# OpenGene/repaq

Hardware: AMD Instinct MI355X
Metric: raw FASTQ MB/s encode+decode (higher is better)
Workload: dtype u8; 1 GPU; configs[2]: synthetic NovaSeq PE150 two files (-i/-I), 2 x 4.01 GB FASTQ (fqgen profile 1, 11200000 pairs, seed 3, N 20 ppm), -k 1000, encode + decode; chunks_per_gpu=3360, parity=unchecked (checked with --full)

## Files before the change

include/rfq_hip.h:

```cpp
#ifndef RFQ_HIP_H
#define RFQ_HIP_H
#include <stddef.h>
#include <stdint.h>
#ifdef __cplusplus
extern "C" {
#endif

#define RFQ_OK              0
#define RFQ_E_NO_DEVICE    -1
#define RFQ_E_HIP          -2
#define RFQ_E_ARG          -3
#define RFQ_E_TEXT         -4
#define RFQ_E_DATA         -5
#define RFQ_E_FORMAT       -6
#define RFQ_E_UNPINNED     -7
#define RFQ_E_NOSPACE      -8
#define RFQ_E_STATE        -9

#define RFQ_SE             0
#define RFQ_PE_TWO_FILES   1
#define RFQ_PE_INTERLEAVED 2

#define RFQ_HEADER_MAX     (17 + 255)

typedef struct rfq_ctx rfq_ctx;

#define RFQ_API __attribute__((visibility("default")))

RFQ_API int         rfq_create(rfq_ctx** out, int device_id);
RFQ_API void        rfq_destroy(rfq_ctx* ctx);
RFQ_API const char* rfq_last_error(const rfq_ctx* ctx);
RFQ_API int         rfq_set_stream(rfq_ctx* ctx, void* hip_stream);

RFQ_API int rfq_set_header(rfq_ctx* ctx, const uint8_t* h_header, size_t header_len);
RFQ_API int rfq_get_header(rfq_ctx* ctx, uint8_t* h_out , size_t* header_len);
RFQ_API void rfq_clear_header(rfq_ctx* ctx);

typedef struct {
    const uint8_t* d_fq1; size_t n1;
    const uint8_t* d_fq2; size_t n2;
    int32_t  paired;
    uint32_t chunk_bases;
    int32_t  final;
    int32_t  emit_header;
    uint64_t file_off1, file_off2;
    uint64_t nolb_from1, nolb_from2;
    uint8_t* d_out; size_t out_cap;
    int32_t  flush_all;
    uint32_t carry_bases;
} rfq_encode_args;

typedef struct {
    const uint8_t* d_rfq;
    size_t   rfq_len;
    uint32_t n_chunks;
    uint64_t n_reads;
    uint64_t n_bases;
    size_t   consumed1, consumed2;
    const uint64_t* h_chunk_off;
    int32_t  input_ended;
    int32_t  reserved;
} rfq_encode_result;

RFQ_API int rfq_encode_batch(rfq_ctx* ctx, const rfq_encode_args* args, rfq_encode_result* res);

typedef struct {
    uint32_t n_chunks;
    uint64_t n_reads;
    size_t   consumed1, consumed2;
    const uint64_t* h_end1;
    const uint64_t* h_end2;
    int32_t  input_ended;
    uint32_t unit_bases;
} rfq_scan_result;
RFQ_API int rfq_scan_batch(rfq_ctx* ctx, const rfq_encode_args* args, rfq_scan_result* res);

typedef struct {
    const uint8_t* d_rfq; size_t n;
    int32_t  has_header;
    int32_t  split_pe;
    int32_t  final;
    int32_t  bug_compat;
    uint8_t* d_out1; size_t cap1;
    uint8_t* d_out2; size_t cap2;
    const uint64_t* h_chunk_off; uint32_t n_chunk_off; uint32_t reserved3;
} rfq_decode_args;

typedef struct {
    const uint8_t* d_fq1; size_t n1;
    const uint8_t* d_fq2; size_t n2;
    uint32_t n_chunks;
    uint64_t n_reads, n_bases;
    size_t   consumed;
} rfq_decode_result;

RFQ_API int rfq_decode_batch(rfq_ctx* ctx, const rfq_decode_args* args, rfq_decode_result* res);

#define RFQ_ROWS_ASCII 0
#define RFQ_ROWS_CODE  1
typedef struct {
    const uint8_t* d_rfq; size_t n;
    int32_t  has_header, final;
    const uint64_t* h_chunk_off; uint32_t n_chunk_off;
    uint32_t row_len;
    int32_t  base_mode;
    uint8_t  qual_offset;
    uint8_t  pad_base, pad_qual;
    uint8_t  reserved;
    uint8_t* d_bases; size_t bases_cap;
    uint8_t* d_quals; size_t quals_cap;
    int32_t* d_lens;  size_t lens_cap;
} rfq_decode_rows_args;
typedef struct {
    uint64_t n_rows, n_bases;
    uint32_t n_chunks, max_len;
    size_t   consumed;
} rfq_decode_rows_result;
RFQ_API int rfq_decode_rows(rfq_ctx* ctx, const rfq_decode_rows_args* args, rfq_decode_rows_result* res);

typedef struct {
    uint64_t n_rows;
    uint32_t row_len;
    int32_t  base_mode;
    uint8_t  qual_offset;
    uint8_t  reserved[3];
    const uint8_t* d_bases;
    const uint8_t* d_quals;
    const int32_t* d_lens;
    const uint8_t* d_names; size_t names_len;
    const uint64_t* d_name_off;
} rfq_rows_in;
typedef struct {
    const uint8_t* d_fq1; size_t n1;
    const uint8_t* d_fq2; size_t n2;
    uint64_t n_reads, n_bases;
} rfq_rows_text_result;
RFQ_API int rfq_rows_to_text(rfq_ctx* ctx, const rfq_rows_in* rows, int32_t paired, uint8_t* d_out1, size_t cap1, uint8_t* d_out2, size_t cap2,
                             int32_t size_only, rfq_rows_text_result* res);
RFQ_API int rfq_encode_rows(rfq_ctx* ctx, const rfq_rows_in* rows, const rfq_encode_args* enc, rfq_encode_result* res);

RFQ_API int rfq_last_timings(const rfq_ctx* ctx, const char** names, float* ms, int cap);

RFQ_API int rfq_dev_malloc(rfq_ctx* ctx, void** d_ptr, size_t n);
RFQ_API int rfq_dev_free(rfq_ctx* ctx, void* d_ptr);
RFQ_API int rfq_copy_h2d(rfq_ctx* ctx, void* d_dst, const void* h_src, size_t n);
RFQ_API int rfq_copy_h2d_async(rfq_ctx* ctx, void* d_dst, const void* h_src, size_t n, uint64_t* ticket);
RFQ_API int rfq_copy_done(rfq_ctx* ctx, uint64_t ticket);
RFQ_API int rfq_copy_sync(rfq_ctx* ctx);
RFQ_API int rfq_copy_d2h(rfq_ctx* ctx, void* h_dst, const void* d_src, size_t n);
RFQ_API int rfq_copy_d2d(rfq_ctx* ctx, void* d_dst, const void* d_src, size_t n);
RFQ_API int rfq_copy_peer(rfq_ctx* ctx, void* d_dst, const rfq_ctx* src_ctx, const void* d_src, size_t n);
RFQ_API int rfq_host_alloc(rfq_ctx* ctx, void** h_ptr, size_t n);
RFQ_API int rfq_host_free(rfq_ctx* ctx, void* h_ptr);
RFQ_API int rfq_host_register(rfq_ctx* ctx, void* h_ptr, size_t n);
RFQ_API int rfq_host_unregister(rfq_ctx* ctx, void* h_ptr);

RFQ_API int rfq_compare_bytes(rfq_ctx* ctx, const void* d_a, const void* d_b, size_t n, uint64_t* first_diff);

RFQ_API int rfq_set_option(rfq_ctx* ctx, const char* name, const char* value);
RFQ_API int rfq_get_option(const rfq_ctx* ctx, const char* name, char* out, size_t cap);
RFQ_API const char* rfq_option_name(int i);

RFQ_API int rfq_selftest_wave(rfq_ctx* ctx, const uint64_t* h_in, uint32_t n_waves, uint64_t* h_out);

RFQ_API const char* rfq_version(void);

#ifdef __cplusplus
}
#endif
#endif
```

repaq_amd/_capi.py:

```python
import ctypes as C
import os

_HERE = os.path.dirname(os.path.abspath(__file__))
DEFAULT_LIB = os.path.join(_HERE, "lib", "librfq_hip.so")

RFQ_OK = 0
SE, PE_TWO_FILES, PE_INTERLEAVED = 0, 1, 2
HEADER_MAX = 17 + 255
U64_MAX = (1 << 64) - 1
ERRORS = {-1: "RFQ_E_NO_DEVICE", -2: "RFQ_E_HIP", -3: "RFQ_E_ARG", -4: "RFQ_E_TEXT", -5: "RFQ_E_DATA", -6: "RFQ_E_FORMAT",
          -7: "RFQ_E_UNPINNED", -8: "RFQ_E_NOSPACE", -9: "RFQ_E_STATE"}


class RfqError(RuntimeError):
    def __init__(self, code, msg):
        super().__init__("%s: %s" % (ERRORS.get(code, code), msg))
        self.code = code
        self.message = msg


class EncodeArgs(C.Structure):
    _fields_ = [("d_fq1", C.c_void_p), ("n1", C.c_size_t), ("d_fq2", C.c_void_p), ("n2", C.c_size_t), ("paired", C.c_int32),
                ("chunk_bases", C.c_uint32), ("final", C.c_int32), ("emit_header", C.c_int32), ("file_off1", C.c_uint64),
                ("file_off2", C.c_uint64), ("nolb_from1", C.c_uint64), ("nolb_from2", C.c_uint64), ("d_out", C.c_void_p), ("out_cap", C.c_size_t),
                ("flush_all", C.c_int32), ("carry_bases", C.c_uint32)]


class EncodeResult(C.Structure):
    _fields_ = [("d_rfq", C.c_void_p), ("rfq_len", C.c_size_t), ("n_chunks", C.c_uint32), ("n_reads", C.c_uint64), ("n_bases", C.c_uint64),
                ("consumed1", C.c_size_t), ("consumed2", C.c_size_t), ("h_chunk_off", C.POINTER(C.c_uint64)),
                ("input_ended", C.c_int32), ("reserved", C.c_int32)]


class ScanResult(C.Structure):
    _fields_ = [("n_chunks", C.c_uint32), ("n_reads", C.c_uint64), ("consumed1", C.c_size_t), ("consumed2", C.c_size_t),
                ("h_end1", C.POINTER(C.c_uint64)), ("h_end2", C.POINTER(C.c_uint64)), ("input_ended", C.c_int32), ("unit_bases", C.c_uint32)]


class DecodeArgs(C.Structure):
    _fields_ = [("d_rfq", C.c_void_p), ("n", C.c_size_t), ("has_header", C.c_int32), ("split_pe", C.c_int32), ("final", C.c_int32), ("bug_compat", C.c_int32),
                ("d_out1", C.c_void_p), ("cap1", C.c_size_t), ("d_out2", C.c_void_p), ("cap2", C.c_size_t),
                ("h_chunk_off", C.POINTER(C.c_uint64)), ("n_chunk_off", C.c_uint32), ("reserved3", C.c_uint32)]


class DecodeResult(C.Structure):
    _fields_ = [("d_fq1", C.c_void_p), ("n1", C.c_size_t), ("d_fq2", C.c_void_p), ("n2", C.c_size_t), ("n_chunks", C.c_uint32),
                ("n_reads", C.c_uint64), ("n_bases", C.c_uint64), ("consumed", C.c_size_t)]


ROWS_ASCII, ROWS_CODE = 0, 1


class DecodeRowsArgs(C.Structure):
    _fields_ = [("d_rfq", C.c_void_p), ("n", C.c_size_t), ("has_header", C.c_int32), ("final", C.c_int32),
                ("h_chunk_off", C.POINTER(C.c_uint64)), ("n_chunk_off", C.c_uint32), ("row_len", C.c_uint32), ("base_mode", C.c_int32),
                ("qual_offset", C.c_uint8), ("pad_base", C.c_uint8), ("pad_qual", C.c_uint8), ("reserved", C.c_uint8),
                ("d_bases", C.c_void_p), ("bases_cap", C.c_size_t), ("d_quals", C.c_void_p), ("quals_cap", C.c_size_t),
                ("d_lens", C.c_void_p), ("lens_cap", C.c_size_t)]


class DecodeRowsResult(C.Structure):
    _fields_ = [("n_rows", C.c_uint64), ("n_bases", C.c_uint64), ("n_chunks", C.c_uint32), ("max_len", C.c_uint32), ("consumed", C.c_size_t)]


class RowsIn(C.Structure):
    _fields_ = [("n_rows", C.c_uint64), ("row_len", C.c_uint32), ("base_mode", C.c_int32), ("qual_offset", C.c_uint8), ("reserved", C.c_uint8 * 3),
                ("d_bases", C.c_void_p), ("d_quals", C.c_void_p), ("d_lens", C.c_void_p), ("d_names", C.c_void_p), ("names_len", C.c_size_t),
                ("d_name_off", C.c_void_p)]


class RowsTextResult(C.Structure):
    _fields_ = [("d_fq1", C.c_void_p), ("n1", C.c_size_t), ("d_fq2", C.c_void_p), ("n2", C.c_size_t), ("n_reads", C.c_uint64), ("n_bases", C.c_uint64)]


_libs = {}


def load(path=None):
    path = path or os.environ.get("RFQ_HIP_LIBRARY") or DEFAULT_LIB
    if path in _libs:
        return _libs[path]
    try:
        import torch
    except Exception:
        pass
    if not os.path.exists(path):
        raise ImportError("librfq_hip.so not found at %s — build it with `python -c 'import __graft_entry__ as g; g.build()'` "
                          "(hipcc --offload-arch=gfx950); repaq_amd has no CPU fallback" % path)
    L = C.CDLL(path)
    L.rfq_version.restype = C.c_char_p
    L.rfq_create.argtypes = [C.POINTER(C.c_void_p), C.c_int]
    L.rfq_destroy.argtypes = [C.c_void_p]
    L.rfq_last_error.argtypes = [C.c_void_p]; L.rfq_last_error.restype = C.c_char_p
    L.rfq_set_stream.argtypes = [C.c_void_p, C.c_void_p]
    L.rfq_set_header.argtypes = [C.c_void_p, C.c_char_p, C.c_size_t]
    L.rfq_get_header.argtypes = [C.c_void_p, C.c_char_p, C.POINTER(C.c_size_t)]
    L.rfq_clear_header.argtypes = [C.c_void_p]; L.rfq_clear_header.restype = None
    L.rfq_encode_batch.argtypes = [C.c_void_p, C.POINTER(EncodeArgs), C.POINTER(EncodeResult)]
    L.rfq_decode_batch.argtypes = [C.c_void_p, C.POINTER(DecodeArgs), C.POINTER(DecodeResult)]
    L.rfq_decode_rows.argtypes = [C.c_void_p, C.POINTER(DecodeRowsArgs), C.POINTER(DecodeRowsResult)]
    L.rfq_rows_to_text.argtypes = [C.c_void_p, C.POINTER(RowsIn), C.c_int32, C.c_void_p, C.c_size_t, C.c_void_p, C.c_size_t, C.c_int32, C.POINTER(RowsTextResult)]
    L.rfq_encode_rows.argtypes = [C.c_void_p, C.POINTER(RowsIn), C.POINTER(EncodeArgs), C.POINTER(EncodeResult)]
    L.rfq_scan_batch.argtypes = [C.c_void_p, C.POINTER(EncodeArgs), C.POINTER(ScanResult)]
    L.rfq_last_timings.argtypes = [C.c_void_p, C.POINTER(C.c_char_p), C.POINTER(C.c_float), C.c_int]
    L.rfq_dev_malloc.argtypes = [C.c_void_p, C.POINTER(C.c_void_p), C.c_size_t]
    L.rfq_dev_free.argtypes = [C.c_void_p, C.c_void_p]
    L.rfq_copy_h2d.argtypes = [C.c_void_p, C.c_void_p, C.c_char_p, C.c_size_t]
    L.rfq_copy_h2d_async.argtypes = [C.c_void_p, C.c_void_p, C.c_void_p, C.c_size_t, C.POINTER(C.c_uint64)]
    L.rfq_copy_done.argtypes = [C.c_void_p, C.c_uint64]
    L.rfq_copy_sync.argtypes = [C.c_void_p]
    L.rfq_copy_d2h.argtypes = [C.c_void_p, C.c_void_p, C.c_void_p, C.c_size_t]
    L.rfq_copy_d2d.argtypes = [C.c_void_p, C.c_void_p, C.c_void_p, C.c_size_t]
    L.rfq_copy_peer.argtypes = [C.c_void_p, C.c_void_p, C.c_void_p, C.c_void_p, C.c_size_t]
    L.rfq_host_alloc.argtypes = [C.c_void_p, C.POINTER(C.c_void_p), C.c_size_t]
    L.rfq_host_free.argtypes = [C.c_void_p, C.c_void_p]
    L.rfq_compare_bytes.argtypes = [C.c_void_p, C.c_void_p, C.c_void_p, C.c_size_t, C.POINTER(C.c_uint64)]
    L.rfq_set_option.argtypes = [C.c_void_p, C.c_char_p, C.c_char_p]
    L.rfq_get_option.argtypes = [C.c_void_p, C.c_char_p, C.c_char_p, C.c_size_t]
    L.rfq_option_name.argtypes = [C.c_int]; L.rfq_option_name.restype = C.c_char_p
    L.rfq_selftest_wave.argtypes = [C.c_void_p, C.POINTER(C.c_uint64), C.c_uint32, C.POINTER(C.c_uint64)]
    _libs[path] = L
    return L


EXPORTS = ["rfq_version", "rfq_create", "rfq_destroy", "rfq_last_error", "rfq_set_stream", "rfq_set_header", "rfq_get_header", "rfq_clear_header",
           "rfq_encode_batch", "rfq_scan_batch", "rfq_decode_batch", "rfq_decode_rows", "rfq_rows_to_text", "rfq_encode_rows", "rfq_last_timings", "rfq_dev_malloc", "rfq_dev_free", "rfq_copy_h2d", "rfq_copy_d2h",
           "rfq_copy_h2d_async", "rfq_copy_done", "rfq_copy_sync",
           "rfq_copy_d2d", "rfq_copy_peer", "rfq_host_alloc", "rfq_host_free", "rfq_compare_bytes", "rfq_selftest_wave", "rfq_set_option", "rfq_get_option", "rfq_option_name", "rfq_host_register", "rfq_host_unregister"]
```

repaq_amd/codec.py:

```python
import ctypes as C

from . import _capi as A
from ._capi import RfqError, SE, PE_TWO_FILES, PE_INTERLEAVED, U64_MAX


class RfqCodec:
    def __init__(self, device=0, library=None):
        self._L = A.load(library)
        h = C.c_void_p()
        rc = self._L.rfq_create(C.byref(h), device)
        if rc != A.RFQ_OK:
            raise RfqError(rc, "rfq_create(device=%d) failed: no usable MI355X / HIP device (there is no CPU fallback)" % device)
        self._h = h

    def close(self):
        if getattr(self, "_h", None):
            self._L.rfq_destroy(self._h)
            self._h = None

    __del__ = close

    def _check(self, rc):
        if rc != A.RFQ_OK:
            raise RfqError(rc, self._L.rfq_last_error(self._h).decode("latin-1"))

    def version(self):
        return self._L.rfq_version().decode()

    def set_stream(self, stream_ptr):
        self._check(self._L.rfq_set_stream(self._h, stream_ptr))

    def set_option(self, name, value=None):
        self._check(self._L.rfq_set_option(self._h, name.encode(), None if value is None else str(value).encode()))

    def get_option(self, name) -> str:
        buf = C.create_string_buffer(64)
        self._check(self._L.rfq_get_option(self._h, name.encode(), buf, 64))
        return buf.value.decode()

    def option_names(self):
        out, i = [], 0
        while True:
            n = self._L.rfq_option_name(i)
            if not n:
                return out
            out.append(n.decode()); i += 1

    def option(self, name, value):
        import contextlib

        @contextlib.contextmanager
        def scope():
            before = self.get_option(name)
            self.set_option(name, value)
            try:
                yield self
            finally:
                self.set_option(name, before or None)
        return scope()

    def selftest_wave(self, lanes):
        n = len(lanes); assert n and n % 64 == 0
        a = (C.c_uint64 * n)(*lanes); o = (C.c_uint64 * (12 * n))()
        self._check(self._L.rfq_selftest_wave(self._h, a, n // 64, o))
        return [list(o[12 * i: 12 * i + 12]) for i in range(n)]

    def setHeader(self, header_bytes: bytes):
        self._check(self._L.rfq_set_header(self._h, header_bytes, len(header_bytes)))

    def clearHeader(self):
        self._L.rfq_clear_header(self._h)

    def header(self) -> bytes:
        buf = C.create_string_buffer(A.HEADER_MAX); n = C.c_size_t()
        self._check(self._L.rfq_get_header(self._h, buf, C.byref(n)))
        return buf.raw[: n.value]

    def encode(self, d_fq1, n1, d_fq2=None, n2=0, paired=SE, chunk_bases=1_000_000, final=True, emit_header=True,
               file_off1=0, file_off2=0, nolb_from1=U64_MAX, nolb_from2=U64_MAX, d_out=None, out_cap=0, flush_all=False):
        a = A.EncodeArgs(d_fq1, n1, d_fq2, n2, paired, chunk_bases, 1 if final else 0, 1 if emit_header else 0,
                         file_off1, file_off2, nolb_from1, nolb_from2, d_out, out_cap, 1 if flush_all else 0, 0)
        r = A.EncodeResult()
        self._check(self._L.rfq_encode_batch(self._h, C.byref(a), C.byref(r)))
        return r

    def scan(self, d_fq1, n1, d_fq2=None, n2=0, paired=SE, chunk_bases=1_000_000, final=True, file_off1=0, file_off2=0, carry_bases=0):
        a = A.EncodeArgs(d_fq1, n1, d_fq2, n2, paired, chunk_bases, 1 if final else 0, 0, file_off1, file_off2, U64_MAX, U64_MAX, None, 0, 0, carry_bases)
        r = A.ScanResult()
        self._check(self._L.rfq_scan_batch(self._h, C.byref(a), C.byref(r)))
        ends1 = [r.h_end1[i] for i in range(r.n_chunks)]
        ends2 = [r.h_end2[i] for i in range(r.n_chunks)] if (paired == PE_TWO_FILES and r.n_chunks) else []
        return r, ends1, ends2

    def decode(self, d_rfq, n, has_header=True, split_pe=False, final=True, d_out1=None, cap1=0, d_out2=None, cap2=0, chunk_off=None, n_chunks=0, bug_compat=False):
        if chunk_off is not None and not isinstance(chunk_off, C.POINTER(C.c_uint64)):
            n_chunks = len(chunk_off) - 1
            chunk_off = C.cast((C.c_uint64 * len(chunk_off))(*chunk_off), C.POINTER(C.c_uint64))
        a = A.DecodeArgs(d_rfq, n, 1 if has_header else 0, 1 if split_pe else 0, 1 if final else 0, 1 if bug_compat else 0, d_out1, cap1, d_out2, cap2,
                         chunk_off if (chunk_off is not None and n_chunks) else None, n_chunks if chunk_off is not None else 0, 0)
        r = A.DecodeResult()
        self._check(self._L.rfq_decode_batch(self._h, C.byref(a), C.byref(r)))
        return r

    def decode_rows(self, d_rfq, n, row_len=0, codes=False, qual_offset=33, pad_base=255, pad_qual=255, d_bases=None, bases_cap=0, d_quals=None, quals_cap=0,
                    d_lens=None, lens_cap=0, has_header=True, final=True, chunk_off=None, n_chunks=0):
        if chunk_off is not None and not isinstance(chunk_off, C.POINTER(C.c_uint64)):
            n_chunks = len(chunk_off) - 1
            chunk_off = C.cast((C.c_uint64 * len(chunk_off))(*chunk_off), C.POINTER(C.c_uint64))
        a = A.DecodeRowsArgs(d_rfq, n, 1 if has_header else 0, 1 if final else 0, chunk_off if (chunk_off is not None and n_chunks) else None,
                             n_chunks if chunk_off is not None else 0, row_len, A.ROWS_CODE if codes else A.ROWS_ASCII, qual_offset, pad_base, pad_qual, 0,
                             d_bases, bases_cap, d_quals, quals_cap, d_lens, lens_cap)
        r = A.DecodeRowsResult()
        self._check(self._L.rfq_decode_rows(self._h, C.byref(a), C.byref(r)))
        return r

    def decode_rows_bytes(self, rfq: bytes, row_len=None, codes=False, qual_offset=33, pad_base=255, pad_qual=255, bases=True, quals=True, lens=True, **kw):
        import numpy as np
        d = self.dev_put(rfq); bufs = []
        try:
            q = self.decode_rows(d, len(rfq), **kw)
            L = max(q.max_len, 1) if row_len is None else int(row_len)
            n = q.n_rows; nb = max(n * L, 1)
            ob = self.dev_put(b"\0" * nb) if bases else None
            oq = self.dev_put(b"\0" * nb) if quals else None
            ol = self.dev_put(b"\0" * max(4 * n, 4)) if lens else None
            bufs = [x for x in (ob, oq, ol) if x is not None]
            r = self.decode_rows(d, len(rfq), row_len=L, codes=codes, qual_offset=qual_offset, pad_base=pad_base, pad_qual=pad_qual,
                                 d_bases=ob, bases_cap=n * L, d_quals=oq, quals_cap=n * L, d_lens=ol, lens_cap=n, **kw)
            n = r.n_rows

            def rows(p):
                return np.frombuffer(self.dev_get(p, n * L), dtype=np.uint8).reshape(n, L) if p is not None else None
            lv = np.frombuffer(self.dev_get(ol, 4 * n), dtype=np.int32) if ol is not None else None
            return n, r.max_len, rows(ob), rows(oq), lv
        finally:
            self.dev_free(d)
            for p in bufs:
                self.dev_free(p)

    @staticmethod
    def _rows_in(n_rows, row_len, d_bases, d_quals, d_lens, d_names, names_len, d_name_off, codes, qual_offset):
        return A.RowsIn(n_rows, row_len, A.ROWS_CODE if codes else A.ROWS_ASCII, qual_offset, (C.c_uint8 * 3)(), d_bases, d_quals, d_lens, d_names, names_len, d_name_off)

    def rows_to_text(self, n_rows, row_len, d_bases, d_quals, d_lens, d_names, names_len, d_name_off, paired=SE, codes=False, qual_offset=33,
                     d_out1=None, cap1=0, d_out2=None, cap2=0, size_only=False):
        a = self._rows_in(n_rows, row_len, d_bases, d_quals, d_lens, d_names, names_len, d_name_off, codes, qual_offset)
        r = A.RowsTextResult()
        self._check(self._L.rfq_rows_to_text(self._h, C.byref(a), paired, d_out1, cap1, d_out2, cap2, 1 if size_only else 0, C.byref(r)))
        return r

    def encode_rows(self, n_rows, row_len, d_bases, d_quals, d_lens, d_names, names_len, d_name_off, paired=SE, codes=False, qual_offset=33,
                    chunk_bases=1_000_000, final=True, emit_header=True, file_off1=0, file_off2=0, nolb_from1=U64_MAX, nolb_from2=U64_MAX,
                    d_out=None, out_cap=0, flush_all=False, d_fq1=None):
        a = self._rows_in(n_rows, row_len, d_bases, d_quals, d_lens, d_names, names_len, d_name_off, codes, qual_offset)
        e = A.EncodeArgs(d_fq1, 0, None, 0, paired, chunk_bases, 1 if final else 0, 1 if emit_header else 0,
                         file_off1, file_off2, nolb_from1, nolb_from2, d_out, out_cap, 1 if flush_all else 0, 0)
        r = A.EncodeResult()
        self._check(self._L.rfq_encode_rows(self._h, C.byref(a), C.byref(e), C.byref(r)))
        return r

    def _put_rows(self, bases, quals, lens, names):
        import numpy as np
        bases = np.ascontiguousarray(bases, dtype=np.uint8); quals = np.ascontiguousarray(quals, dtype=np.uint8)
        lens = np.ascontiguousarray(lens, dtype=np.int32)
        n = int(lens.shape[0]); L = int(bases.shape[1]) if bases.ndim == 2 else 0
        assert bases.shape == quals.shape == (n, L) and len(names) == n and L >= 1, "bases / quals [n, L], lens [n], n names"
        off = np.zeros(n + 1, dtype=np.uint64)
        if n:
            off[1:] = np.cumsum(np.fromiter((len(x) for x in names), dtype=np.uint64, count=n))
        blob = b"".join(names)
        ptrs = [self.dev_put(x) for x in (bases.tobytes(), quals.tobytes(), lens.tobytes(), blob, off.tobytes())]
        return ptrs, (n, L, ptrs[0], ptrs[1], ptrs[2], ptrs[3], len(blob), ptrs[4])

    def rows_to_text_bytes(self, bases, quals, lens, names, paired=SE, codes=False, qual_offset=33):
        ptrs, rows = self._put_rows(bases, quals, lens, names)
        try:
            r = self.rows_to_text(*rows, paired=paired, codes=codes, qual_offset=qual_offset)
            a = self.dev_get(r.d_fq1, r.n1) if r.n1 else b""
            b = self.dev_get(r.d_fq2, r.n2) if (paired == PE_TWO_FILES and r.n2) else b""
            return (a, b) if paired == PE_TWO_FILES else a
        finally:
            for p in ptrs:
                self.dev_free(p)

    def encode_rows_bytes(self, bases, quals, lens, names, paired=SE, chunk_bases=1_000_000, codes=False, qual_offset=33, **kw) -> bytes:
        ptrs, rows = self._put_rows(bases, quals, lens, names)
        try:
            r = self.encode_rows(*rows, paired=paired, codes=codes, qual_offset=qual_offset, chunk_bases=chunk_bases, **kw)
            return self.dev_get(r.d_rfq, r.rfq_len) if r.rfq_len else b""
        finally:
            for p in ptrs:
                self.dev_free(p)

    def first_diff(self, d_a, d_b, n) -> int:
        out = C.c_uint64(0)
        self._check(self._L.rfq_compare_bytes(self._h, d_a, d_b, n, C.byref(out)))
        return out.value

    def timings(self):
        names = (C.c_char_p * 32)(); ms = (C.c_float * 32)()
        n = self._L.rfq_last_timings(self._h, names, ms, 32)
        return [(names[i].decode(), ms[i]) for i in range(n)]

    def dev_put(self, data: bytes):
        p = C.c_void_p()
        self._check(self._L.rfq_dev_malloc(self._h, C.byref(p), max(len(data), 1) + 64))
        self._check(self._L.rfq_copy_h2d(self._h, p, data, len(data)))
        return p

    def dev_get(self, d_ptr, n) -> bytes:
        buf = C.create_string_buffer(max(n, 1))
        self._check(self._L.rfq_copy_d2h(self._h, buf, d_ptr, n))
        return buf.raw[:n]

    def dev_free(self, p):
        self._L.rfq_dev_free(self._h, p)

    def encode_bytes(self, fq1: bytes, fq2: bytes = b"", paired=SE, chunk_bases=1_000_000, **kw) -> bytes:
        d1 = self.dev_put(fq1); d2 = self.dev_put(fq2) if paired == PE_TWO_FILES else None
        try:
            r = self.encode(d1, len(fq1), d2, len(fq2) if d2 else 0, paired, chunk_bases, **kw)
            return self.dev_get(r.d_rfq, r.rfq_len) if r.rfq_len else b""
        finally:
            self.dev_free(d1)
            if d2:
                self.dev_free(d2)

    def decode_bytes(self, rfq: bytes, split_pe=False, out_caps=None, **kw):
        d = self.dev_put(rfq); o1 = o2 = None
        try:
            if out_caps is not None:
                o1 = self.dev_put(b"\0" * max(int(out_caps[0]), 1)); o2 = self.dev_put(b"\0" * max(int(out_caps[1]), 1)) if split_pe else None
                kw = dict(kw, d_out1=o1, cap1=int(out_caps[0]), d_out2=o2, cap2=int(out_caps[1]) if split_pe else 0)
            r = self.decode(d, len(rfq), split_pe=split_pe, **kw)
            a = self.dev_get(r.d_fq1, r.n1) if r.n1 else b""
            b = self.dev_get(r.d_fq2, r.n2) if (split_pe and r.n2) else b""
            return (a, b) if split_pe else a
        finally:
            self.dev_free(d)
            if o1 is not None: self.dev_free(o1)
            if o2 is not None: self.dev_free(o2)


def nolb_threshold(file_size: int, ends_with_newline: bool) -> int:
    if file_size == 0:
        return U64_MAX
    if file_size % (1 << 20) == 0:
        return file_size
    if ends_with_newline:
        return U64_MAX
    return ((file_size - 1) >> 20) << 20
```

repaq_amd/csrc/dec/emit_tiles.h:

```cpp
#pragma once
#define E3_QCAP 10240u
#define E3_SHARED_OK 1
#define E3_ALIGNED 1
#define E3_PROBE_WRAP 0
#define E3_PREFETCH 0
#define E3_L2PF 1
#define E3_N1BIG 13312u
struct __attribute__((packed, aligned(1))) GU16d { uint32_t a, b, c, d; };
struct __attribute__((packed, aligned(1))) GU8d { uint32_t a, b; };
struct __attribute__((packed, aligned(1))) GU4d { uint32_t a; };
struct __attribute__((packed, aligned(1))) GU2d { uint16_t a; };
__device__ __forceinline__ void e3_copy(uint8_t* __restrict__ dst, const uint8_t* src, uint32_t n, uint32_t g0, uint32_t gs, int pat, uint32_t dch) {
    if (n >= 16u) {
        const uint32_t ng = (n + 15u) >> 4;
        for (uint32_t g = g0; g < ng; g += gs) {
            uint32_t p0 = 16u * g; if (p0 + 16u > n) p0 = n - 16u;
            uint32_t w[4]; lds_get16(src, p0, w);
            if (pat >= (int)p0 && pat < (int)p0 + 16) { const int b = pat - (int)p0; const uint32_t sh = 8u * (uint32_t)(b & 3); uint32_t& x = w[b >> 2];
                    x = (x & ~(0xFFu << sh)) | ((dch & 0xFFu) << sh); }
            GU16d v; v.a = w[0]; v.b = w[1]; v.c = w[2]; v.d = w[3]; *(GU16d*)(dst + p0) = v;
        }
    } else if (g0 == 0 && n) {
        uint32_t w[4]; lds_get16(src, 0, w);
        if (pat >= 0 && pat < 16) { const uint32_t sh = 8u * (uint32_t)(pat & 3); uint32_t& x = w[pat >> 2]; x = (x & ~(0xFFu << sh)) | ((dch & 0xFFu) << sh); }
        uint8_t* q = dst;
        if (n & 8u) { GU8d v; v.a = w[0]; v.b = w[1]; *(GU8d*)q = v; q += 8; w[0] = w[2]; w[1] = w[3]; }
        if (n & 4u) { GU4d v; v.a = w[0]; *(GU4d*)q = v; q += 4; w[0] = w[1]; }
        if (n & 2u) { GU2d v; v.a = (uint16_t)w[0]; *(GU2d*)q = v; q += 2; w[0] >>= 16; }
        if (n & 1u) *q = (uint8_t)w[0];
    }
}
__device__ __forceinline__ uint32_t e3_rev2x16(uint32_t v) { v = bswap32(v); v = ((v >> 4) & 0x0F0F0F0Fu) | ((v & 0x0F0F0F0Fu) << 4);
        return ((v >> 2) & 0x33333333u) | ((v & 0x33333333u) << 2); }
__device__ __forceinline__ uint32_t e3_rev1x16(uint32_t v) {
    v = ((v >> 8) & 0xFFu) | ((v & 0xFFu) << 8); v = ((v >> 4) & 0x0F0Fu) | ((v & 0x0F0Fu) << 4);
    v = ((v >> 2) & 0x3333u) | ((v & 0x3333u) << 2); return ((v >> 1) & 0x5555u) | ((v & 0x5555u) << 1);
}
__device__ __forceinline__ uint32_t e3_from(int t, int i) { const int k = t - 4 * i; return k <= 0 ? 0xFFFFFFFFu : (k >= 4 ? 0u : 0xFFFFFFFFu << (8 * k)); }
__device__ __forceinline__ uint32_t e3_align(uint32_t hi, uint32_t lo, int bytes) { return (uint32_t)((((unsigned long long)hi << 32) | lo) >> (8 * bytes)); }
template <bool IMPL, uint32_t N1CAP = ET_N1CAP, bool SHARED = false> __global__ void __launch_bounds__(256, (N1CAP == ET_N1CAP && !(SHARED && E3_PREFETCH)) ? 5 : 4) k_dec_emit3(const uint8_t* __restrict__ img,
        const DChunk* __restrict__ CH, const DevHeader* __restrict__ D, DFused F,
                           uint64_t img_bytes, int split, uint8_t* __restrict__ out1, uint64_t cap1, uint8_t* __restrict__ out2, uint64_t cap2, DecStatus* st,
                           const plist_t* __restrict__ plist, const unsigned long long* __restrict__ loff, const uint32_t* __restrict__ nent, const uint32_t* __restrict__ cellidx,
                           uint32_t ncell, uint32_t nstr, uint32_t kshift, unsigned long long list_cap) {
    __shared__ uint4 t_q4[E3_QCAP / 16 + 6];
    constexpr uint32_t NB = (SHARED && E3_PREFETCH) ? 2u : 1u;
    __shared__ uint4 t_pk4[NB][E3_QCAP / 64 + 6];
    __shared__ uint32_t t_nb[E3_QCAP / 32 + 8];
    __shared__ uint4 t_mid4_[NB][64 * E3_MIDROW / 16 + 5], t_n14_[(SHARED ? 256u : N1CAP) / 16 + 5], t_n24_[(SHARED ? 256u : ET_N2CAP) / 16 + 5], t_st4[(SHARED ? 256u : ET_STCAP) / 16 + 4];
    uint4* const t_n14 = t_n14_ + 1; uint4* const t_n24 = t_n24_ + 1;
    __shared__ unsigned long long s_loff[NPOS_SLOT + 2]; __shared__ uint32_t s_nent[NPOS_SLOT + 2], s_val[NPOS_SLOT + 2];
    __shared__ uint32_t s_g[2][NPOS_SLOT + 2], s_kb[2][NPOS_SLOT + 2];
    const uint32_t c = blockIdx.y; const DChunk d = CH[c]; const uint8_t* cp = img + d.off;
    const uint32_t fl = d.flags, hf = D->flags, f = d.rbase; const bool il = (fl & C_PE_INTERLEAVED) != 0;
    constexpr bool implied_n = IMPL;
    const uint32_t nq4 = (D->n_base_qual & 0xFFu) * 0x01010101u, dpos = D->name2_diff_pos, dch = D->name2_diff_char;
    const int l = lane_id(), w = (int)uni32((uint32_t)wave_id()); const uint32_t tid = threadIdx.x;
    const size_t fp = (size_t)f + c;
    const U4 tb = F.tbase[c];
    const uint32_t K = 1u << kshift, pshift = 8u - kshift, P = 1u << pshift;
    uint32_t per = (d.reads + gridDim.x - 1) / gridDim.x; per = (per + K - 1u) & ~(K - 1u);
    const uint32_t rs = blockIdx.x * per; const uint32_t re = rs + per < d.reads ? rs + per : d.reads;
    if (rs >= re) return;
    if (list_cap && ((st->err & (uint32_t)(DE_CORRUPT | DE_CORRUPT_OV | DE_LIST_ALIAS | DE_E3_RETRY)) || st->list_need > list_cap)) return;
    const bool raw = !SHARED && (hf & H_DONT_QUAL) != 0, bycol = SHARED || (!raw && (hf & H_QUAL_BY_COL));
    const uint32_t nn = bycol ? (D->n_normal < NPOS_SLOT ? D->n_normal : NPOS_SLOT) : 0u; const bool hasn = (hf & H_N_POS) != 0;
    const uint32_t T = nn + (hasn ? 1u : 0u);
    const uint32_t major4 = (D->major & 0xFFu) * 0x01010101u;
    const uint32_t qlen_c = F.pql[fp + d.reads], slen_c = F.sdl[fp + d.reads];
    const bool same1 = SHARED || (fl & C_NAME1_SAME) != 0, same2 = SHARED || (fl & C_NAME2_SAME) != 0, same3 = SHARED || (fl & C_STRAND_SAME) != 0;
    if (tid < T) { const uint32_t jj = tid < nn ? tid : D->n_normal; const size_t t_ = (size_t)c * nstr + jj; s_loff[tid] = loff[t_]; s_nent[tid] = nent[t_];
            s_val[tid] = tid < nn ? (uint32_t)D->normal[tid] : (uint32_t)'N'; }
    uint32_t nrec = 0; const uint8_t* xrec = nullptr;
    if (bycol && 4ull * D->n_normal <= d.qual_size) {
        const uint8_t* qp = cp + d.o_qual; uint64_t off = 4ull * D->n_normal;
        for (uint32_t i = 0; i < D->n_normal; i++) off += ld_u32(qp + 4 * i);
        off = uni64(off);
        if (off <= d.qual_size) { nrec = (uint32_t)((d.qual_size - off) / 5); xrec = qp + off; }
    }
    auto cell_lookup = [&](uint32_t t, uint32_t qpos, uint32_t spos, bool bound) -> uint32_t {
        const uint32_t jj = t < nn ? t : D->n_normal; uint32_t cell = ((t < nn ? qpos : spos) + (bound ? E3_QCAP : 0u)) / POS2_CELL + (bound ? 1u : 0u);
        if (cell >= ncell) return bound ? 0xFFFFFFFFu : cellidx[((size_t)c * nstr + jj) * ncell + ncell - 1u];
        return cellidx[((size_t)c * nstr + jj) * ncell + cell];
    };
    struct TileP { uint32_t q0, q1, s0, s1, a7, a8, a9, e7, e8, e9; };
    auto tile_params = [&](uint32_t r0, uint32_t r1) -> TileP {
        TileP t; t.q0 = uni32(F.pql[fp + r0]); t.q1 = uni32(F.pql[fp + r1]);
        t.s0 = uni32(F.sdl[fp + r0]); t.s1 = uni32(F.sdl[fp + r1]);
        if constexpr (SHARED) { t.a7 = t.a8 = t.a9 = t.e7 = t.e8 = t.e9 = 0u; }
        else { const U4 a = F.pvl[fp + r0], b = F.pvl[fp + r1];
               t.a7 = uni32(a.a); t.a8 = uni32(a.b); t.a9 = uni32(a.c); t.e7 = uni32(b.a); t.e8 = uni32(b.b); t.e9 = uni32(b.c); }
        return t;
    };
    constexpr bool PF = SHARED && E3_PREFETCH;
    uint32_t cur = rs, pb = 0; uint32_t l2pf = 0; (void)l2pf;
    TileP tp_cur = tile_params(cur, cur + K < re ? cur + K : re);
    if (tid < T) { s_g[0][tid] = cell_lookup(tid, tp_cur.q0, tp_cur.s0, false); s_kb[0][tid] = cell_lookup(tid, tp_cur.q0, tp_cur.s0, true); }
    {
        const uint64_t ib = d.off;
        if (same1) span_dma<1>(make_span(t_n14, img, ib + d.o_n1, ib + d.o_n1 + d.n1_size, img_bytes, true));
        if (same2) span_dma<1>(make_span(t_n24, img, ib + d.o_n2, ib + d.o_n2 + d.n2_size, img_bytes, true));
        if (same3) span_dma<1>(make_span(t_st4, img, ib + d.o_st, ib + d.o_st + d.st_size, img_bytes, true));
    }
    const uint32_t jj = tid >> pshift, j = ((jj << 1) & (K - 1u)) | (jj >> (kshift - 1u)), part = tid & (P - 1u);
    struct TileD { uint64_t n1a, n1e, n2a, n2e, sta, ste, pka, pke, rqa, rqe; };
    auto tile_spans = [&](const TileP& tp) -> TileD {
        TileD t; const uint64_t ib = d.off;
        t.n1a = ib + d.o_n1 + (same1 ? 0u : tp.a7); t.n1e = same1 ? t.n1a + d.n1_size : ib + d.o_n1 + tp.e7;
        t.n2a = ib + d.o_n2 + (same2 ? 0u : tp.a8); t.n2e = same2 ? t.n2a + d.n2_size : ib + d.o_n2 + tp.e8;
        t.sta = ib + d.o_st + (same3 ? 0u : tp.a9); t.ste = same3 ? t.sta + d.st_size : ib + d.o_st + tp.e9;
        t.pka = ib + d.o_seq + (tp.s0 >> 2); t.pke = ib + d.o_seq + ((tp.s1 + 3u) >> 2); { const uint64_t pend = ib + d.o_seq + d.seq_size; if (t.pke > pend) t.pke = pend;
                if (t.pka > t.pke) t.pka = t.pke; }
        t.rqa = ib + d.o_qual + tp.q0; t.rqe = ib + d.o_qual + tp.q1; { const uint64_t qend = ib + d.o_qual + d.qual_size; if (t.rqe > qend) t.rqe = qend;
                if (t.rqa > t.rqe) t.rqa = t.rqe; }
        return t;
    };
    auto tile_fits = [&](const TileP& tp) -> bool {
        return tp.q1 - tp.q0 <= E3_QCAP && (same1 || tp.e7 - tp.a7 + 32u <= N1CAP) && (same2 || tp.e8 - tp.a8 + 32u <= ET_N2CAP) && (same3 || tp.e9 - tp.a9 + 32u <= ET_STCAP);
    };
    auto stage = [&](const TileD& t, uint32_t g0_, uint32_t g1_, uint32_t bsel) {
        if (raw) span_dma<(int)((E3_QCAP / 16 + 4 + 255) / 256)>(make_span(t_q4 + 1, img, t.rqa, t.rqe, img_bytes, true));
        if (w == 0) span_dma_wave<(int)((E3_QCAP / 64 + 4 + 63) / 64), PF>(make_span(t_pk4[bsel], img, t.pka, t.pke, img_bytes, true), l);
        else if (w == 1) span_dma_wave<(int)((64 * E3_MIDROW / 16 + 4 + 63) / 64), PF>(make_span(t_mid4_[bsel] + 1, F.mid, (uint64_t)g0_ * E3_MIDROW, (uint64_t)g1_ * E3_MIDROW, ~0ull >> 1, true), l);
        else if (w == 2) { if (!same1) span_dma_wave<(int)((N1CAP / 16 + 4 + 63) / 64)>(make_span(t_n14, img, t.n1a, t.n1e, img_bytes, true), l); }
        else { if (!same2) span_dma_wave<(int)((ET_N2CAP / 16 + 4 + 63) / 64)>(make_span(t_n24, img, t.n2a, t.n2e, img_bytes, true), l);
               if (!same3) span_dma_wave<(int)((ET_STCAP / 16 + 4 + 63) / 64)>(make_span(t_st4, img, t.sta, t.ste, img_bytes, true), l); }
    };
    struct ReadM { uint32_t len, md, prevlen, sdl, pql, tx; int ov; U4 p4; uint8_t n1, n2, sl; };
    auto load_read = [&](uint32_t cur_, uint32_t cnt_) -> ReadM {
        ReadM m; m.len = m.n1 = m.n2 = m.sl = m.md = m.prevlen = m.sdl = m.pql = m.tx = 0; m.ov = 0; m.p4.a = m.p4.b = m.p4.c = m.p4.d = 0;
        const uint32_t r = cur_ + j;
        if (j < cnt_) {
            const uint32_t g_ = f + r; const uint2 t2 = F.tpl[g_];
            m.sdl = F.sdl[fp + r];
            if constexpr (!SHARED) m.p4 = F.pvl[fp + r];
            m.tx = t2.x; m.pql = F.pql[fp + r];
            m.len = F.len[g_]; m.ov = F.ov[g_]; m.prevlen = (r & 1u) ? F.len[g_ - 1] : 0u;
            m.n1 = cp[d.o_n1lens + ((fl & C_NAME1_LEN_SAME) ? 0u : r)]; m.n2 = (hf & H_NAME2) ? cp[d.o_n2lens + ((fl & C_NAME2_LEN_SAME) ? 0u : r)] : 0u;
            m.sl = cp[d.o_stlens + ((fl & C_STRAND_LEN_SAME) ? 0u : r)]; m.md = t2.y;
        }
        return m;
    };
    struct ListS { uint32_t fe[8], fv[8], pn[2], nk0, nke, t, base, k0, ke, val; const plist_t* p; };
    auto ls_open = [&](ListS& L, uint32_t pb_, uint32_t t_) {
        const uint32_t g_ = uni32(s_g[pb_][t_]), b_ = uni32(s_kb[pb_][t_]), n_ = uni32(s_nent[t_]);
        L.k0 = g_ == 0xFFFFFFFFu ? 0u : g_; L.ke = g_ == 0xFFFFFFFFu ? 0u : (b_ < n_ ? b_ : n_); L.base = 0;
        L.val = uni32(s_val[t_]); L.p = plist + uni64(s_loff[t_]);
    };
    auto ls_round = [&](ListS& L, uint32_t pb_, uint32_t& e_, uint32_t& v_) {
        while (L.t < nn && L.k0 + L.base >= L.ke) { L.t += 4u; if (L.t < nn) ls_open(L, pb_, L.t); }
        if (L.t < nn) { const uint32_t kk = L.k0 + L.base + (uint32_t)l; if (kk < L.ke) e_ = L.p[kk]; v_ = L.val; L.base += 64u; }
    };
    auto load_lists = [&](uint32_t pb_) -> ListS {
        ListS L; L.t = (uint32_t)w; L.base = L.k0 = L.ke = L.val = 0; L.p = plist;
        if (L.t < nn) ls_open(L, pb_, L.t); else L.t = nn;
#pragma unroll
        for (int i = 0; i < 8; i++) { L.fe[i] = 0xFFFFFFFFu; L.fv[i] = 0; ls_round(L, pb_, L.fe[i], L.fv[i]); }
        L.pn[0] = L.pn[1] = 0xFFFFFFFFu; L.nk0 = 0xFFFFFFFFu; L.nke = 0;
        if (hasn) {
            L.nk0 = s_g[pb_][nn]; L.nke = s_kb[pb_][nn]; if (L.nke > s_nent[nn]) L.nke = s_nent[nn];
            const plist_t* lp = plist + s_loff[nn];
#pragma unroll
            for (int i = 0; i < 2; i++) { const uint32_t kk = L.nk0 + tid + 256u * (uint32_t)i; if (L.nk0 != 0xFFFFFFFFu && kk < L.nke) L.pn[i] = lp[kk]; }
        }
        return L;
    };
    __syncthreads();
    ReadM mN; ListS lN;
    if constexpr (PF) {
        if (tile_fits(tp_cur)) { const uint32_t cnt0 = re - cur < K ? re - cur : K; stage(tile_spans(tp_cur), f + cur, f + cur + cnt0, 0u); mN = load_read(cur, cnt0); lN = load_lists(0u); }
        else { mN = load_read(cur, 0u); lN = load_lists(0u); }
    }
    while (cur < re) {
        const uint32_t cnt = re - cur < K ? re - cur : K, g0 = f + cur, g1 = g0 + cnt;
        const TileP tp = tp_cur; const uint32_t q0 = tp.q0, q1 = tp.q1, s0 = tp.s0, s1 = tp.s1;
        if (!tile_fits(tp)) { if (tid == 0) atomicOr(&st->err, (uint32_t)DE_E3_RETRY); break; }
        const TileD td = tile_spans(tp); const uint32_t bs = PF ? pb : 0u;
        const uint64_t n1a = td.n1a, n2a = td.n2a, sta = td.sta, pka = td.pka, pke = td.pke, rqa = td.rqa;
        if constexpr (!PF) { stage(td, g0, g1, 0u); mN = load_read(cur, cnt); lN = load_lists(pb); }
        const ReadM m = mN; ListS ls = lN;
        if (bycol) { uint4* qt = t_q4 + 1; const uint32_t ng = (q1 - q0 + 15u) >> 4;
                for (uint32_t i = tid; i < ng; i += blockDim.x) qt[i] = make_uint4(major4, major4, major4, major4); }
        for (uint32_t i = tid; i < ((s1 - s0 + 31u) >> 5) + 1u; i += blockDim.x) t_nb[i] = 0;
        const uint32_t r = cur + j; const bool on = j < cnt; const bool odd = (r & 1u) != 0, rc = il && odd, to2 = split && odd;
        const uint32_t len = m.len, n1 = m.n1, n2 = m.n2, sl = m.sl, md = m.md, prevlen = m.prevlen; const int ov = m.ov;
        uint32_t sp = 0, qp_ = 0, o7 = 0, o8 = 0, o9 = 0, toff = 0;
        if (on) { sp = m.sdl - s0; qp_ = m.pql - q0; toff = (to2 ? tb.b : tb.a) + m.tx; if constexpr (!SHARED) { o7 = m.p4.a - tp.a7; o8 = m.p4.b - tp.a8; o9 = m.p4.c - tp.a9; } }
        const uint32_t nxt = cur + cnt; TileP tp_n = tp;
        if (nxt < re) tp_n = tile_params(nxt, nxt + K < re ? nxt + K : re);
#ifndef RFQ_SIMT_EMULATION
        if constexpr (PF) __builtin_amdgcn_s_waitcnt(0x0F70);
#endif
        __syncthreads();
#if E3_L2PF && !defined(RFQ_SIMT_EMULATION)
        if (SHARED) asm volatile("" :: "v"(l2pf));
#endif
        uint8_t* const q_t = (uint8_t*)(t_q4 + 1) + (raw ? (uint32_t)(rqa & 15ull) : 0u);
        const uint8_t* const pk = (const uint8_t*)t_pk4[bs] + (uint32_t)(pka & 15ull);
        const uint4* const t_mid4 = t_mid4_[bs] + 1;
        const uint32_t have = (uint32_t)(pke - pka), sbit0 = 2u * (s0 & 3u);
        {
#pragma unroll
            for (int i = 0; i < 8; i++) { const uint32_t p = plist_pos(ls.fe[i], q0); if (p < q1) q_t[p - q0] = (uint8_t)ls.fv[i]; }
            while (ls.t < nn) {
                uint32_t e_[4], v_[4];
#pragma unroll
                for (int i = 0; i < 4; i++) { e_[i] = 0xFFFFFFFFu; v_[i] = 0; ls_round(ls, pb, e_[i], v_[i]); }
#pragma unroll
                for (int i = 0; i < 4; i++) { const uint32_t p = plist_pos(e_[i], q0); if (p < q1) q_t[p - q0] = (uint8_t)v_[i]; }
            }
            if (nrec) for (uint32_t i = tid; i < nrec; i += blockDim.x) { const uint8_t* rr = xrec + 5ull * i; const uint32_t pos = ld_u32(rr + 1);
                    if (pos >= q0 && pos < q1 && pos < qlen_c) q_t[pos - q0] = rr[0]; }
            if (hasn) {
                const uint32_t send = s1 < slen_c ? s1 : slen_c;
#pragma unroll
                for (int i = 0; i < 2; i++) { const uint32_t p = plist_pos(ls.pn[i], s0); if (p < send) atomicOr(&t_nb[(p - s0) >> 5], 1u << ((p - s0) & 31u)); }
                if (ls.nk0 != 0xFFFFFFFFu && ls.nk0 + 512u < ls.nke) { const plist_t* lp = plist + s_loff[nn];
                        for (uint32_t kk = ls.nk0 + 512u + tid; kk < ls.nke; kk += 256u) { const uint32_t p = plist_pos((uint32_t)lp[kk], s0);
                        if (p < send) atomicOr(&t_nb[(p - s0) >> 5], 1u << ((p - s0) & 31u)); } }
            }
        }
        if (nxt < re && tid < T) { s_g[pb ^ 1u][tid] = cell_lookup(tid, tp_n.q0, tp_n.s0, false); s_kb[pb ^ 1u][tid] = cell_lookup(tid, tp_n.q0, tp_n.s0, true); }
        __syncthreads();
        if constexpr (PF) {
            if (nxt < re) {
                const uint32_t cntn = re - nxt < K ? re - nxt : K;
                if (tile_fits(tp_n)) { stage(tile_spans(tp_n), f + nxt, f + nxt + cntn, pb ^ 1u); mN = load_read(nxt, cntn); lN = load_lists(pb ^ 1u); }
            }
        }
#if E3_L2PF && !defined(RFQ_SIMT_EMULATION)
        if (SHARED && nxt < re) {
            const uint32_t cntn = re - nxt < K ? re - nxt : K; const TileD tn = tile_spans(tp_n);
            const uint8_t* pb_ = nullptr; uint32_t nbytes = 0;
            const uint32_t grp = tid >> 5, li = tid & 31u; uint32_t line = li;
            if (grp == 0) { pb_ = img + tn.pka; nbytes = (uint32_t)(tn.pke - tn.pka); }
            else if (grp == 1) { pb_ = F.mid + (size_t)(f + nxt) * E3_MIDROW; nbytes = cntn * E3_MIDROW; }
            else if (grp == 2) {
                const uint32_t a = li >> 2; line = li & 3u;
                if (a == 0) { pb_ = (const uint8_t*)(F.tpl + f + nxt); nbytes = cntn * 8u; }
                else if (a == 1) { pb_ = (const uint8_t*)(F.sdl + fp + nxt); nbytes = cntn * 4u; }
                else if (a == 2) { pb_ = (const uint8_t*)(F.pql + fp + nxt); nbytes = cntn * 4u; }
                else if (a == 3) { pb_ = (const uint8_t*)(F.len + f + nxt); nbytes = cntn * 4u; }
                else if (a == 4) { pb_ = (const uint8_t*)(F.ov + f + nxt); nbytes = cntn * 4u; }
            }
            else {
                const uint32_t t_ = grp - 3u, st_ = t_ < 4u ? t_ : nn;
                if ((t_ < 4u && t_ < nn) || (t_ == 4u && hasn)) {
                    const uint32_t g_ = s_g[pb ^ 1u][st_], b_ = s_kb[pb ^ 1u][st_], n_ = s_nent[st_]; const uint32_t ke = b_ < n_ ? b_ : n_;
                    if (g_ != 0xFFFFFFFFu && g_ < ke) { pb_ = (const uint8_t*)(plist + s_loff[st_] + g_); nbytes = (ke - g_) * (uint32_t)sizeof(plist_t); }
                }
            }
            if (nbytes) {
                const uint8_t* const a0 = (const uint8_t*)((uintptr_t)pb_ & ~(uintptr_t)127); const uint32_t span = (uint32_t)(pb_ - a0) + nbytes;
                if (128u * line < span) { const uint8_t* q = a0 + 128u * line; asm volatile("global_load_dword %0, %1, off" : "=v"(l2pf) : "v"(q)); }
            }
        }
#endif
        if (on) {
            uint8_t* const rec = (to2 ? out2 : out1) + (E3_PROBE_WRAP ? (toff & (uint32_t)E3_PROBE_WRAP) : toff); const uint64_t capo = to2 ? cap2 : cap1;
            const uint32_t e0 = n1 + md + n2, oseq = e0 + 1u, ost = oseq + len + 1u, oq = ost + sl + 1u, total = oq + len + 1u;
            if ((uint64_t)toff + total > capo) { if (part == 0) atomicOr(&st->err, 1u << 31); }
            else {
                const uint32_t L = e0 + 1u; const bool nfast = L >= 16u, jfast = sl == 1u && len >= 16u;
                const uint8_t* const src1 = (const uint8_t*)t_n14 + (uint32_t)(n1a & 15ull) + (same1 ? 0u : o7);
                const uint8_t* const src2 = (const uint8_t*)t_mid4 + (uint32_t)(((uint64_t)g0 * E3_MIDROW) & 15ull) + E3_MIDROW * j;
                const uint8_t* const src3 = (const uint8_t*)t_n24 + (uint32_t)(n2a & 15ull) + (same2 ? 0u : o8);
                const uint8_t* const src4 = (const uint8_t*)t_st4 + (uint32_t)(sta & 15ull) + (same3 ? 0u : o9);
                const int pat2 = (same2 && rc && dch != 0 && dpos < n2) ? (int)dpos : -1;
                if (nfast) {
                    const uint32_t ngl = (L + 15u) >> 4;
                    for (uint32_t gi = part; gi < ngl; gi += P) {
                        uint32_t p0 = 16u * gi; if (p0 + 16u > L) p0 = L - 16u;
                        const int t1 = (int)n1 - (int)p0, t2 = t1 + (int)md, t3 = t2 + (int)n2;
                        uint32_t w[4] = { 0, 0, 0, 0 }, x[4];
                        if (t1 > 0) lds_get16(src1 + p0, 0, w);
                        if (t1 < 16 && t2 > 0 && md) { lds_get16(src2 - t1, 0, x);
#pragma unroll
                            for (int i = 0; i < 4; i++) { const uint32_t m = e3_from(t1, i); w[i] = (w[i] & ~m) | (x[i] & m); } }
                        if (t2 < 16 && t3 > 0 && n2) { lds_get16(src3 - t2, 0, x);
                            if (pat2 >= 0) { const int b = t2 + pat2; if (b >= 0 && b < 16) { const uint32_t sh = 8u * (uint32_t)(b & 3); uint32_t& y = x[b >> 2];
                                    y = (y & ~(0xFFu << sh)) | ((dch & 0xFFu) << sh); } }
#pragma unroll
                            for (int i = 0; i < 4; i++) { const uint32_t m = e3_from(t2, i); w[i] = (w[i] & ~m) | (x[i] & m); } }
                        if (t3 == 15) w[3] = (w[3] & 0x00FFFFFFu) | 0x0A000000u;
                        GU16d v; v.a = w[0]; v.b = w[1]; v.c = w[2]; v.d = w[3]; *(GU16d*)(rec + p0) = v;
                    }
                } else {
                    if (part == 0) e3_copy(rec, src1, n1, 0, 1, -1, 0);
                    else if (part == 1 % P) e3_copy(rec + n1, src2, md, 0, 1, -1, 0);
                    if (part == 2 % P) e3_copy(rec + n1 + md, src3, n2, 0, 1, pat2, dch);
                    if (part == 3 % P) rec[e0] = '\n';
                }
                if (!jfast && part == 3 % P) { e3_copy(rec + ost, src4, sl, 0, 1, -1, 0); rec[ost - 1u] = '\n'; rec[oq - 1u] = '\n'; rec[total - 1u] = '\n'; }
                const uint32_t xa = ov < 0 ? len - (uint32_t)(-ov) : len; const uint32_t A = ov > 0 ? sp - (uint32_t)ov : sp, Bs = sp - prevlen;
                auto fetch = [&](uint32_t si, uint32_t& cw, uint32_t& nw) {
                    const uint32_t bit = sbit0 + 2u * si, byte = bit >> 3; const unsigned long long v = lds_get8(pk, byte);
                    cw = (uint32_t)(v >> (bit & 7u));
                    const uint32_t nb_ = lds_get4((const uint8_t*)t_nb, (si >> 3)) >> (si & 7u); nw = nb_ & 0xFFFFu;
                    if (byte + 5u > have) { uint32_t lim_ = 4u * have > sbit0 / 2u + si ? 4u * have - sbit0 / 2u - si : 0u;
                            if (lim_ < 16u) nw |= (0xFFFFu << lim_) & 0xFFFFu; }
                };
                auto group_q = [&](uint32_t k0, uint32_t (&qw)[4]) {
                    const uint32_t pa = rc ? len - k0 - 16u : k0;
                    lds_get16(q_t, qp_ + pa, qw);
                    if (rc) { const uint32_t x0 = bswap32(qw[3]), x1 = bswap32(qw[2]), x2 = bswap32(qw[1]), x3 = bswap32(qw[0]); qw[0] = x0; qw[1] = x1; qw[2] = x2; qw[3] = x3; }
                };
                auto group_s = [&](uint32_t k0, const uint32_t (&qw)[4], uint32_t (&sw)[4]) {
                    const uint32_t pa = rc ? len - k0 - 16u : k0;
                    uint32_t cw, nw;
                    if (pa + 16u <= xa) fetch(A + pa, cw, nw);
                    else if (pa >= xa) fetch(Bs + (pa - xa), cw, nw);
                    else { uint32_t c2, n2_; const uint32_t t1 = xa - pa; fetch(A + pa, cw, nw); fetch(Bs, c2, n2_);
                            cw = (cw & ((1u << (2u * t1)) - 1u)) | (c2 << (2u * t1)); nw = (nw & ((1u << t1) - 1u)) | ((n2_ << t1) & 0xFFFFu); }
                    if (rc) { cw = ~e3_rev2x16(cw); if (nw) nw = e3_rev1x16(nw); }
#pragma unroll
                    for (int i = 0; i < 4; i++) { const uint32_t b = (cw >> (8 * i)) & 0xFFu, y = (b | (b << 12)) & 0x000F000Fu, idx = (y | (y << 6)) & 0x03030303u;
                            sw[i] = __builtin_amdgcn_perm(0u, 0x43544147u, idx); }
                    if (nw) {
#pragma unroll
                        for (int i = 0; i < 4; i++) { const uint32_t mk = ((((nw >> (4 * i)) & 0xFu) * 0x00204081u) & 0x01010101u) * 0xFFu;
                                sw[i] = (sw[i] & ~mk) | (0x4E4E4E4Eu & mk); }
                    }
                    if (implied_n) {
#pragma unroll
                        for (int i = 0; i < 4; i++) { const uint32_t mk = eq_bytes_full(qw[i], nq4); sw[i] = (sw[i] & ~mk) | (0x4E4E4E4Eu & mk); }
                    }
                };
                auto group = [&](uint32_t k0, uint32_t (&qw)[4], uint32_t (&sw)[4]) { group_q(k0, qw); group_s(k0, qw, sw); };
                auto st16 = [&](uint32_t at, const uint32_t (&x)[4]) { GU16d v; v.a = x[0]; v.b = x[1]; v.c = x[2]; v.d = x[3]; *(GU16d*)(rec + at) = v; };
                auto put = [&](uint32_t at_q, uint32_t at_s, const uint32_t (&qw)[4], const uint32_t (&sw)[4], bool both) {
                    GU16d v;
                    if (both) { v.a = qw[0]; v.b = qw[1]; v.c = qw[2]; v.d = qw[3]; *(GU16d*)(rec + at_q) = v; }
                    v.a = sw[0]; v.b = sw[1]; v.c = sw[2]; v.d = sw[3]; *(GU16d*)(rec + at_s) = v;
                };
                if (len >= 16u) {
                    uint32_t qw[4], sw[4];
                    const bool al = E3_ALIGNED && len >= 32u;
                    uint32_t rs, tail_part;
                    if (al) {
                        const uint32_t hs = (16u - (uint32_t)((uintptr_t)(rec + oseq) & 15u)) & 15u, hq = (16u - (uint32_t)((uintptr_t)(rec + oq) & 15u)) & 15u;
                        const uint32_t nts = ((len - hs) >> 4) + (hs ? 1u : 0u), ntq = ((len - hq) >> 4) + (hq ? 1u : 0u);
                        for (uint32_t t = part; t < nts; t += P) { const uint32_t k0 = hs ? (t ? hs + 16u * (t - 1u) : 0u) : 16u * t;
                                if (implied_n) group_q(k0, qw);
                                group_s(k0, qw, sw); st16(oseq + k0, sw); }
                        const uint32_t p2 = (part + P - (nts & (P - 1u))) & (P - 1u);
                        for (uint32_t t = p2; t < ntq; t += P) { const uint32_t k0 = hq ? (t ? hq + 16u * (t - 1u) : 0u) : 16u * t; group_q(k0, qw); st16(oq + k0, qw); }
                        rs = (len - hs) & 15u; tail_part = (nts + ntq) & (P - 1u);
                        if (!jfast && tail_part == part) {
                            const uint32_t rq = (len - hq) & 15u;
                            if (rs || rq) { group(len - 16u, qw, sw); if (rq) st16(oq + len - 16u, qw); if (rs) st16(oseq + len - 16u, sw); }
                        }
                    } else {
                        const uint32_t nfull = len >> 4;
                        for (uint32_t gi = part; gi < nfull; gi += P) { group(16u * gi, qw, sw); put(oq + 16u * gi, oseq + 16u * gi, qw, sw, true); }
                        rs = len & 15u; tail_part = nfull & (P - 1u);
                        if (!jfast && tail_part == part && rs) { group(len - 16u, qw, sw); put(oq + len - 16u, oseq + len - 16u, qw, sw, true); }
                    }
                    if (jfast && tail_part == part) {
                        group(len - 16u, qw, sw);
                        {
                            if (rs > 13u) put(0u, oseq + len - 16u, qw, sw, false);
                            const uint32_t jd = 0x000A000Au | ((uint32_t)src4[0] << 8);
                            uint32_t qs[4], ss[4];
                            ss[0] = e3_align(sw[1], sw[0], 3); ss[1] = e3_align(sw[2], sw[1], 3); ss[2] = e3_align(sw[3], sw[2], 3); ss[3] = e3_align(jd, sw[3], 3);
                            qs[0] = e3_align(qw[1], qw[0], 1); qs[1] = e3_align(qw[2], qw[1], 1); qs[2] = e3_align(qw[3], qw[2], 1); qs[3] = e3_align(0x0Au, qw[3], 1);
                            put(oq + len - 15u, oseq + len - 13u, qs, ss, true);
                        }
                    }
                } else if (part == 0) {
                    for (uint32_t k = 0; k < len; k++) {
                        const uint32_t p = rc ? len - 1u - k : k, si = p < xa ? A + p : Bs + (p - xa);
                        const uint32_t bit = sbit0 + 2u * si, byte = bit >> 3; const uint32_t code = byte < have ? (pk[byte] >> (bit & 7u)) & 3u : 0u;
                        const bool isn = byte >= have || ((t_nb[si >> 5] >> (si & 31u)) & 1u);
                        const uint8_t q = q_t[qp_ + p]; uint8_t b = isn ? (uint8_t)'N' : (uint8_t)("GATC"[rc ? 3u - code : code]);
                        if (implied_n && q == (uint8_t)(nq4 & 0xFFu)) b = 'N';
                        rec[oseq + k] = b; rec[oq + k] = q;
                    }
                }
            }
        }
        __syncthreads();
        cur += cnt; pb ^= 1u; tp_cur = tp_n;
    }
}
```

repaq_amd/csrc/dec/read_table.h:

```cpp
#pragma once
struct DReadTab {
    uint32_t* len; uint32_t* chunk; int32_t* ov; U4* pvin; U4* pv; uint32_t* pq; U4* tin; U4* tp;
    uint8_t* mid;
};
__device__ __forceinline__ uint32_t dec_read_len(const uint8_t* cp, const DChunk& d, uint32_t rlb, uint32_t r) {
    const uint8_t* p = cp + d.o_readlens + (size_t)((d.flags & C_READ_LEN_SAME) ? 0u : r) * rlb;
    return rlb == 1 ? p[0] : (rlb == 2 ? ld_u16(p) : ld_u32(p));
}
__global__ void k_dec_readtab(const uint8_t* __restrict__ img, const DChunk* __restrict__ CH, const DevHeader* __restrict__ D, DReadTab R, DecStatus* st) {
    const DChunk d = CH[blockIdx.y]; const uint32_t r = blockIdx.x * blockDim.x + threadIdx.x;
    if (r >= d.reads) return;
    const uint8_t* cp = img + d.off; const uint32_t g = d.rbase + r, fl = d.flags, hf = D->flags;
    const uint32_t len = dec_read_len(cp, d, D->read_len_bytes, r);
    U4 v;
    v.a = (fl & C_NAME1_SAME) ? 0u : cp[d.o_n1lens + ((fl & C_NAME1_LEN_SAME) ? 0u : r)];
    v.b = ((hf & H_NAME2) && !(fl & C_NAME2_SAME)) ? cp[d.o_n2lens + ((fl & C_NAME2_LEN_SAME) ? 0u : r)] : 0u;
    v.c = (fl & C_STRAND_SAME) ? 0u : cp[d.o_stlens + ((fl & C_STRAND_LEN_SAME) ? 0u : r)];
    int ov = 0; uint32_t stored = len;
    if ((fl & C_PE_INTERLEAVED) && (hf & H_PE_OVERLAP) && (r & 1u)) {
        ov = (int)(int8_t)cp[d.o_ov + r / 2] - D->overlap_shift;
        const uint32_t a = (uint32_t)(ov < 0 ? -ov : ov);
        const uint32_t prevlen = dec_read_len(cp, d, D->read_len_bytes, r - 1);
        if (a > len || a > prevlen) { atomicOr(&st->err, (uint32_t)DE_CORRUPT); ov = 0; } else stored = len - a;
    }
    v.d = stored;
    R.len[g] = len; R.chunk[g] = blockIdx.y; R.ov[g] = ov; R.pvin[g] = v;
}
#define E3_MIDROW 32u
struct DFused {
    const uint32_t* len; const int32_t* ov;
    const uint32_t* pql;
    const U4* pvl;
    const uint32_t* sdl;
    const uint2* tpl;
    const U4* tbase;
    const uint8_t* mid;
};
__global__ void __launch_bounds__(256) k_dec_readtab2(const uint8_t* __restrict__ img, const DChunk* __restrict__ CH, const DevHeader* __restrict__ D,
                                                      uint32_t* __restrict__ len_o, int32_t* __restrict__ ov_o, uint32_t* __restrict__ pql, U4* __restrict__ pvl, uint32_t* __restrict__ sdl, DecStatus* st) {
    const uint32_t c = blockIdx.x; const DChunk d = CH[c];
    const uint8_t* cp = img + d.off; const uint32_t fl = d.flags, hf = D->flags, rlb = D->read_len_bytes, shift = (uint32_t)D->overlap_shift;
    const bool ovl = (fl & C_PE_INTERLEAVED) && (hf & H_PE_OVERLAP);
    const size_t fp = (size_t)d.rbase + c;
    U4 carry; carry.a = carry.b = carry.c = carry.d = 0; uint32_t qcarry = 0, bad = 0;
    for (uint32_t r0 = 0; r0 < d.reads; r0 += 4u * blockDim.x) {
        const uint32_t rb = r0 + 4u * threadIdx.x;
        U4 v[4]; uint32_t ln[4]; U4 sum; sum.a = sum.b = sum.c = sum.d = 0; uint32_t qsum = 0;
#pragma unroll
        for (int i = 0; i < 4; i++) {
            const uint32_t r = rb + (uint32_t)i; v[i].a = v[i].b = v[i].c = v[i].d = 0; ln[i] = 0;
            if (r < d.reads) {
                const uint32_t len = dec_read_len(cp, d, rlb, r);
                v[i].a = (fl & C_NAME1_SAME) ? 0u : cp[d.o_n1lens + ((fl & C_NAME1_LEN_SAME) ? 0u : r)];
                v[i].b = ((hf & H_NAME2) && !(fl & C_NAME2_SAME)) ? cp[d.o_n2lens + ((fl & C_NAME2_LEN_SAME) ? 0u : r)] : 0u;
                v[i].c = (fl & C_STRAND_SAME) ? 0u : cp[d.o_stlens + ((fl & C_STRAND_LEN_SAME) ? 0u : r)];
                int ov = 0; uint32_t stored = len;
                if (ovl && (r & 1u)) {
                    ov = (int)(int8_t)cp[d.o_ov + r / 2] - (int)shift;
                    const uint32_t a = (uint32_t)(ov < 0 ? -ov : ov);
                    const uint32_t prevlen = dec_read_len(cp, d, rlb, r - 1);
                    if (a > len || a > prevlen) { bad = 1; ov = 0; } else stored = len - a;
                }
                v[i].d = stored; ln[i] = len;
                len_o[(size_t)d.rbase + r] = len; ov_o[(size_t)d.rbase + r] = ov;
            }
            sum = sum + v[i]; qsum += ln[i];
        }
        U4 tot; uint32_t qtot;
        U4 run = carry + block_excl_sum<U4>(sum, &tot); uint32_t qrun = qcarry + block_excl_sum<uint32_t>(qsum, &qtot);
#pragma unroll
        for (int i = 0; i < 4; i++) { const uint32_t r = rb + (uint32_t)i; if (r < d.reads) { if (pvl) pvl[fp + r] = run; sdl[fp + r] = run.d; pql[fp + r] = qrun; } run = run + v[i]; qrun += ln[i]; }
        carry = carry + tot; qcarry += qtot;
    }
    if (threadIdx.x == 0) { if (pvl) pvl[fp + d.reads] = carry; sdl[fp + d.reads] = carry.d; pql[fp + d.reads] = qcarry; }
    if (__any(bad != 0) && lane_id() == 0) atomicOr(&st->err, (uint32_t)DE_CORRUPT_OV);
}
__global__ void k_dec_bases(const DChunk* __restrict__ CH, DReadTab R, uint64_t* __restrict__ qbase, uint64_t* __restrict__ sbase, uint32_t n_chunks) {
    const uint32_t c = blockIdx.x * blockDim.x + threadIdx.x;
    if (c < n_chunks) { const uint32_t f = CH[c].rbase; qbase[c] = ((uint64_t)R.pq[f] & ~63ull) + 64ull * c; sbase[c] = ((uint64_t)R.pv[f].d & ~63ull) + 64ull * c; }
}

__device__ __forceinline__ uint32_t ld_word_lim(const uint8_t* p, const uint8_t* lim);
__global__ void k_dec_unpack(const uint8_t* __restrict__ img, const DChunk* __restrict__ CH, DReadTab R, const uint64_t* __restrict__ sbase, uint8_t* __restrict__ sdec,
        uint64_t img_bytes) {
    auto unpack4v = [](uint32_t b) -> uint32_t {
        const uint32_t y = (b | (b << 12)) & 0x000F000Fu, idx = (y | (y << 6)) & 0x03030303u;
        return __builtin_amdgcn_perm(0u, 0x43544147u, idx);
    };
    const DChunk d = CH[blockIdx.y]; const uint32_t f = d.rbase;
    const uint32_t n = R.pv[f + d.reads].d - R.pv[f].d;
    const uint8_t* src = img + d.off + d.o_seq; uint8_t* dst = sdec + sbase[blockIdx.y]; const uint8_t* lim = img + img_bytes;
    const uint32_t ngroups = (n + 15) / 16, NT = gridDim.x * blockDim.x;
    const uint32_t ph = (uint32_t)((uintptr_t)src & 3u); const uint8_t* sa = src - ph; const uint32_t sh = ph * 8u;
    for (uint32_t g0 = blockIdx.x * blockDim.x + threadIdx.x; g0 < ngroups; g0 += 4 * NT) {
        uint32_t lo[4], hi[4];
#pragma unroll
        for (int u = 0; u < 4; u++) { const uint32_t gi = g0 + (uint32_t)u * NT; lo[u] = hi[u] = 0; if (gi < ngroups) { lo[u] = ld_word_lim(sa + 4 * (size_t)gi, lim);
                if (ph) hi[u] = ld_word_lim(sa + 4 * (size_t)gi + 4, lim); } }
#pragma unroll
        for (int u = 0; u < 4; u++) {
            const uint32_t gi = g0 + (uint32_t)u * NT; if (gi >= ngroups) continue;
            const uint32_t pk = ph ? (uint32_t)((((uint64_t)hi[u] << 32) | lo[u]) >> sh) : lo[u];
            uint32_t w[4];
#pragma unroll
            for (int k = 0; k < 4; k++) { const uint32_t i = 4 * gi + (uint32_t)k; w[k] = i < d.seq_size ? unpack4v((pk >> (8 * k)) & 0xFFu) : 0x4E4E4E4Eu; }
            if (16 * gi + 16 <= n) *(uint4*)(dst + 16 * (size_t)gi) = make_uint4(w[0], w[1], w[2], w[3]);
            else for (uint32_t p = 16 * gi; p < n; p++) dst[p] = (uint8_t)(w[(p >> 2) & 3u] >> (8 * (p & 3u)));
        }
    }
}
```

repaq_amd/csrc/dec/text_len.h:

```cpp
#pragma once
__device__ __forceinline__ uint32_t dec_digits(uint32_t v) { uint32_t n = 1; while (v >= 10) { v /= 10; n++; } return n; }
__device__ __forceinline__ uint32_t dec_put(uint8_t* dst, uint32_t v) { const uint32_t n = dec_digits(v); for (uint32_t k = 0; k < n; k++) { dst[n - 1 - k] = (uint8_t)('0' + v % 10); v /= 10; } return n; }
__device__ __forceinline__ uint32_t mid_put(uint8_t* buf, uint32_t k, uint32_t cap, uint32_t v) {
    if (v >= 100000000u || k + 9u > cap) { buf[k] = ':'; return 1u + dec_put(buf + k + 1u, v); }
    const uint32_t hi = v / 10000u, lo = v - hi * 10000u;
    const uint32_t a = mul24(hi, 5243u) >> 19, b = hi - mul24(a, 100u), c = mul24(lo, 5243u) >> 19, d = lo - mul24(c, 100u);
    const uint32_t P = a | (b << 16), Q = c | (d << 16);
    const uint32_t pt = ((P * 103u) >> 10) & 0x000F000Fu, po = P - pt * 10u, qt = ((Q * 103u) >> 10) & 0x000F000Fu, qo = Q - qt * 10u;
    const unsigned long long dg = (unsigned long long)(pt | (po << 8)) | ((unsigned long long)(qt | (qo << 8)) << 32);
    const uint32_t lz = dg ? (uint32_t)(__ffsll((long long)dg) - 1) >> 3 : 7u, n = 8u - lz;
    const unsigned long long asc = (dg | 0x3030303030303030ull) >> (8u * lz);
    LdsU8 w; w.a = (asc << 8) | 0x3Aull; *(LdsU8*)(buf + k) = w;
    if (n == 8u) buf[k + 8u] = (uint8_t)(asc >> 56);
    return 1u + n;
}
struct DName { uint32_t n1, n2, st, lane, tile, x, y; };
__device__ __forceinline__ DName dec_name_parts(const uint8_t* cp, const DChunk& d, const DevHeader* D, const uint32_t* xv, const uint32_t* yv, uint32_t r) {
    const uint32_t fl = d.flags, hf = D->flags; DName m;
    m.n1 = cp[d.o_n1lens + ((fl & C_NAME1_LEN_SAME) ? 0u : r)];
    m.n2 = (hf & H_NAME2) ? cp[d.o_n2lens + ((fl & C_NAME2_LEN_SAME) ? 0u : r)] : 0u;
    m.st = cp[d.o_stlens + ((fl & C_STRAND_LEN_SAME) ? 0u : r)];
    const uint32_t xy = (fl & C_PE_INTERLEAVED) ? r / 2 : r;
    m.lane = (hf & H_LANE) ? cp[d.o_lanes + ((fl & C_LANE_SAME) ? 0u : xy)] : 0u;
    m.tile = (hf & H_TILE) ? ld_u16(cp + d.o_tiles + 2 * (size_t)((fl & C_TILE_SAME) ? 0u : xy)) : 0u;
    m.x = (hf & H_X) ? xv[d.rbase + xy] : 0u; m.y = (hf & H_Y) ? yv[d.rbase + xy] : 0u;
    return m;
}
__device__ __forceinline__ uint32_t dec_textlen_one(const uint8_t* __restrict__ img, const DChunk& d, const DevHeader* __restrict__ D, const DReadTab& R,
                                                    const uint32_t* __restrict__ xv, const uint32_t* __restrict__ yv, int split, uint32_t r, bool& second, uint8_t* buf ) {
    const uint8_t* cp = img + d.off; const uint32_t g = d.rbase + r, hf = D->flags;
    const DName m = dec_name_parts(cp, d, D, xv, yv, r);
    uint32_t k = 0;
    { unsigned long long* z = (unsigned long long*)buf; z[0] = z[1] = z[2] = z[3] = z[4] = 0ull; }
    if (hf & H_LANE) k += mid_put(buf, k, 39u, m.lane);
    if (hf & H_TILE) k += mid_put(buf, k, 39u, m.tile);
    if (hf & H_X) k += mid_put(buf, k, 39u, m.x);
    if (hf & H_Y) k += mid_put(buf, k, 39u, m.y);
    buf[39] = (uint8_t)k;
    { const unsigned long long* z = (const unsigned long long*)buf; unsigned long long* mp = (unsigned long long*)(R.mid + (size_t)g * 40);
      const unsigned long long a0 = z[0], a1 = z[1], a2 = z[2], a3 = z[3], a4 = z[4]; mp[0] = a0; mp[1] = a1; mp[2] = a2; mp[3] = a3; mp[4] = a4; }
    const uint32_t nl = m.n1 + m.n2 + k;
    const uint32_t len = R.len[g]; const uint32_t text = nl + 1 + len + 1 + m.st + 1 + len + 1;
    second = split && (r & 1u);
    U4 t; t.a = second ? 0u : text; t.b = second ? text : 0u; t.c = 0; t.d = 0;
    R.tin[g] = t;
    return text;
}
__global__ void k_dec_textlen(const uint8_t* __restrict__ img, const DChunk* __restrict__ CH, const DevHeader* __restrict__ D, DReadTab R,
                              const uint32_t* __restrict__ xv, const uint32_t* __restrict__ yv, int split, DecStatus* st) {
    const DChunk d = CH[blockIdx.y]; const uint32_t r = blockIdx.x * blockDim.x + threadIdx.x;
    if (blockIdx.x * blockDim.x >= d.reads) return;
    uint32_t text = 0; bool second = false;
    __shared__ unsigned long long s_mid[256 * 5];
    if (r < d.reads) text = dec_textlen_one(img, d, D, R, xv, yv, split, r, second, (uint8_t*)(s_mid + 5u * threadIdx.x));
    __shared__ unsigned long long s_t[2][4];
    const unsigned long long s1 = wave_sum<unsigned long long>(second ? 0ull : (unsigned long long)text), s2 = wave_sum<unsigned long long>(second ? (unsigned long long)text : 0ull);
    if (lane_id() == 0) { s_t[0][wave_id()] = s1; s_t[1][wave_id()] = s2; }
    __syncthreads();
    if (threadIdx.x == 0) {
        unsigned long long a = 0, b = 0; for (uint32_t i = 0; i < (blockDim.x >> 6); i++) { a += s_t[0][i]; b += s_t[1][i]; }
        const uint32_t slot = (blockIdx.y * 7u + blockIdx.x) & 63u;
        if (a) atomicAdd((unsigned long long*)&st->text_slots[0][slot], a);
        if (b) atomicAdd((unsigned long long*)&st->text_slots[1][slot], b);
    }
}
__global__ void __launch_bounds__(256) k_dec_textlen2(const uint8_t* __restrict__ img, const DChunk* __restrict__ CH, const DevHeader* __restrict__ D, const uint32_t* __restrict__ len_i,
                                                      uint8_t* __restrict__ mid, const uint32_t* __restrict__ xv, const uint32_t* __restrict__ yv, int split,
                                                      uint2* __restrict__ tpl, U4* __restrict__ ctext, DecStatus* st) {
    __shared__ unsigned long long s_mid[256 * 4];
    const uint32_t c = blockIdx.x; const DChunk d = CH[c]; const uint8_t* cp = img + d.off; const uint32_t hf = D->flags;
    unsigned long long carry = 0, sum1 = 0, sum2 = 0;
    for (uint32_t r0 = 0; r0 < d.reads; r0 += blockDim.x) {
        const uint32_t r = r0 + threadIdx.x; unsigned long long mine = 0; uint32_t k = 0; bool second = false;
        if (r < d.reads) {
            const size_t g = (size_t)d.rbase + r;
            const DName m = dec_name_parts(cp, d, D, xv, yv, r);
            uint8_t* buf = (uint8_t*)(s_mid + 4u * threadIdx.x);
            { unsigned long long* z = (unsigned long long*)buf; z[0] = z[1] = z[2] = z[3] = 0ull; }
            if (hf & H_LANE) k += mid_put(buf, k, E3_MIDROW, m.lane);
            if (hf & H_TILE) k += mid_put(buf, k, E3_MIDROW, m.tile);
            if (hf & H_X) k += mid_put(buf, k, E3_MIDROW, m.x);
            if (hf & H_Y) k += mid_put(buf, k, E3_MIDROW, m.y);
            { const unsigned long long* z = (const unsigned long long*)buf; unsigned long long* mp = (unsigned long long*)(mid + g * E3_MIDROW);
              const unsigned long long a0 = z[0], a1 = z[1], a2 = z[2], a3 = z[3]; mp[0] = a0; mp[1] = a1; mp[2] = a2; mp[3] = a3; }
            const uint32_t len = len_i[g]; const uint32_t text = m.n1 + m.n2 + k + 1 + len + 1 + m.st + 1 + len + 1;
            second = split && (r & 1u);
            mine = second ? ((unsigned long long)text << 32) : (unsigned long long)text;
        }
        unsigned long long tot; const unsigned long long ex = carry + block_excl_sum<unsigned long long>(mine, &tot);
        if (r < d.reads) tpl[(size_t)d.rbase + r] = make_uint2(second ? (uint32_t)(ex >> 32) : (uint32_t)ex, k);
        sum1 += tot & 0xFFFFFFFFull; sum2 += tot >> 32;
        carry = (sum1 & 0xFFFFFFFFull) | (sum2 << 32);
    }
    if (threadIdx.x == 0) {
        U4 t; t.a = (uint32_t)sum1; t.b = (uint32_t)sum2; t.c = 0; t.d = 0; ctext[c] = t;
        const uint32_t slot = (c * 7u) & 63u;
        if (sum1) atomicAdd((unsigned long long*)&st->text_slots[0][slot], sum1);
        if (sum2) atomicAdd((unsigned long long*)&st->text_slots[1][slot], sum2);
    }
}
```

repaq_amd/csrc/rfq_decode.hip:

```cpp
#include "rfq_ctx.h"
#include "rfq_decode_kernels.h"
#include <algorithm>
#include <cstring>
#include <cstdlib>

int rfq_upload_header(rfq_ctx* c, const uint8_t* h, size_t n);

enum DecBuf {
    DB_CHUNKS = 80, DB_STATUS, DB_LEN, DB_CHUNKID, DB_OV, DB_PVIN, DB_PV, DB_PQ, DB_TIN, DB_TP, DB_QBASE, DB_SBASE, DB_QDEC, DB_SDEC, DB_XV, DB_YV, DB_SCAN, DB_MID, DB_SEGF, DB_SEGA, DB_SEGN, DB_SEGS, DB_SEGP, DB_OFFT, DB_CELL, DB_SEGK, DB_NENT, DB_LOFF, DB_PLIST, DB_GWCAND, DB_GWLIST, DB_GWCNT, DB_GWLAND, DB_PQL, DB_PVL, DB_TPL, DB_CTEXT, DB_TBASE, DB_SDL, DB_END
};
static_assert(DB_END <= 120, "rfq_ctx::b too small");

#define RFQ_RANGE_TOO_BIG 2
struct DecRange { const DChunk* CH; uint32_t n_chunks, n_reads, max_reads, max_stream, max_npos, max_len, max_bases, max_nrec, max_one, pieces, piece_avg, piece_n1;
        uint64_t bases; };
static int dec_table_expanded(rfq_ctx* ctx, const rfq_decode_args* a, const DecRange& g, DReadTab& R, bool text, uint32_t* total_bases, U4* pv_tot) {
    hipStream_t S = ctx->stream; DBuf* B = ctx->b; const DevHeader* D = ctx->d_hdr.as<DevHeader>(); DecStatus* dst = B[DB_STATUS].as<DecStatus>();
    const uint32_t n_chunks = g.n_chunks, n_reads = g.n_reads, max_reads = std::max(g.max_reads, 1u);
    const size_t nr = (size_t)n_reads + 2, nc = (size_t)n_chunks + 2;
    HIPCHK(ctx, B[DB_CHUNKID].ensure(nr * 4));
    HIPCHK(ctx, B[DB_PVIN].ensure(nr * 16)); HIPCHK(ctx, B[DB_PV].ensure(nr * 16)); HIPCHK(ctx, B[DB_PQ].ensure(nr * 4));
    if (text) { HIPCHK(ctx, B[DB_TIN].ensure(nr * 16)); HIPCHK(ctx, B[DB_TP].ensure(nr * 16)); }
    HIPCHK(ctx, B[DB_QBASE].ensure(nc * 8)); HIPCHK(ctx, B[DB_SBASE].ensure(nc * 8));
    HIPCHK(ctx, B[DB_SCAN].ensure((nr / SCAN_TILE + 2) * 16 + 1024));
    R.chunk = B[DB_CHUNKID].as<uint32_t>();
    R.pvin = B[DB_PVIN].as<U4>(); R.pv = B[DB_PV].as<U4>(); R.pq = B[DB_PQ].as<uint32_t>();
    R.tin = text ? B[DB_TIN].as<U4>() : nullptr; R.tp = text ? B[DB_TP].as<U4>() : nullptr;
    hipLaunchKernelGGL(k_dec_readtab, dim3((max_reads + 255) / 256, n_chunks), dim3(256), 0, S, a->d_rfq, g.CH, D, R, dst);
    KCHK(ctx, "k_dec_readtab");
    scan_exclusive<uint32_t>(S, R.len, R.pq, n_reads, B[DB_SCAN].as<uint32_t>(), 1);
    scan_exclusive<U4>(S, R.pvin, R.pv, n_reads, B[DB_SCAN].as<U4>(), 1);
    HIPCHK(ctx, ctx->fetch(total_bases, R.pq + n_reads, 4, S));
    HIPCHK(ctx, ctx->fetch(pv_tot, R.pv + n_reads, 16, S));
    DecStatus h2; HIPCHK(ctx, ctx->fetch(&h2, dst, sizeof h2, S)); HIPCHK(ctx, ctx->fetch_sync(S));
    ctx->timer.end(S);
    if (h2.err & DE_CORRUPT) return rfq_fail(ctx, RFQ_E_FORMAT, "corrupt overlap buffer");
    return RFQ_OK;
}
struct DecExpanded { uint64_t* qbase; uint64_t* sbase; uint8_t* qdec; uint8_t* sdec; size_t qbytes, sbytes; };
static int dec_streams_expanded(rfq_ctx* ctx, const rfq_decode_args* a, const DecRange& g, const DReadTab& R, uint32_t total_bases, const U4& pv_tot, bool coords,
                                DecExpanded* E) {
    hipStream_t S = ctx->stream; DBuf* B = ctx->b; const DevHeader& HH = ctx->h_hdr; const DevHeader* D = ctx->d_hdr.as<DevHeader>();
    DecStatus* dst = B[DB_STATUS].as<DecStatus>(); const DChunk* CH = g.CH; const uint32_t n_chunks = g.n_chunks; const size_t nc = (size_t)n_chunks + 2;
    const bool rle_h = !(HH.flags & (H_DONT_QUAL | H_QUAL_BY_COL));
    ctx->timer.begin("streams", S);
    const size_t qbytes = (size_t)total_bases + 64 * nc + 256, sbytes = (size_t)pv_tot.d + 64 * nc + 256;
    HIPCHK(ctx, B[DB_QDEC].ensure(qbytes)); HIPCHK(ctx, B[DB_SDEC].ensure(sbytes));
    uint64_t* const qbase = B[DB_QBASE].as<uint64_t>(); uint64_t* const sbase = B[DB_SBASE].as<uint64_t>();
    uint8_t* const qdec = B[DB_QDEC].as<uint8_t>(); uint8_t* const sdec = B[DB_SDEC].as<uint8_t>();
    hipLaunchKernelGGL(k_dec_bases, dim3((n_chunks + 255) / 256), dim3(256), 0, S, CH, R, qbase, sbase, n_chunks);
    const bool forked = ctx->aux_ready();
    hipStream_t A = forked ? ctx->aux : S;
    if (forked) { HIPCHK(ctx, hipEventRecord(ctx->ev_fork, S)); HIPCHK(ctx, hipStreamWaitEvent(A, ctx->ev_fork, 0)); }
    const uint32_t bpc = std::max(1u, std::min(64u, 4096u / n_chunks));
    hipStream_t F = forked ? ctx->aux2 : S;
    if (forked) HIPCHK(ctx, hipStreamWaitEvent(F, ctx->ev_fork, 0));
    hipLaunchKernelGGL(k_dec_fill, dim3((uint32_t)std::min<size_t>(8192, (qbytes / 16 + 255) / 256 + 1)), dim3(256), 0, F, qdec, (uint64_t)qbytes, D);
    if (forked) HIPCHK(ctx, hipEventRecord(ctx->ev_f, F));
    if (coords) hipLaunchKernelGGL(k_dec_coords, dim3(2, n_chunks), dim3(64), 0, S, a->d_rfq, CH, D, B[DB_XV].as<uint32_t>(), B[DB_YV].as<uint32_t>());
    if ((HH.flags & H_N_POS) || ((HH.flags & H_QUAL_BY_COL) && !(HH.flags & H_DONT_QUAL))) {
        const bool bycol = (HH.flags & H_QUAL_BY_COL) && !(HH.flags & H_DONT_QUAL), hasn = (HH.flags & H_N_POS) != 0;
        const uint32_t nn = bycol ? std::min<uint32_t>(HH.n_normal, NPOS_SLOT) : 0u, nstr = HH.n_normal + 1;
        const uint32_t mq = nn ? g.max_stream / POS_SEG + 1 : 0u, mn = hasn ? g.max_npos / POS_SEG + 1 : 0u, maxseg = std::max(1u, std::max(mq, mn));
        const size_t nseg = (size_t)n_chunks * nstr * maxseg;
        HIPCHK(ctx, B[DB_SEGF].ensure(nseg + 16)); HIPCHK(ctx, B[DB_SEGA].ensure(nseg * 16 + 16)); HIPCHK(ctx, B[DB_SEGN].ensure((size_t)n_chunks * nstr * 4 + 16));
        HIPCHK(ctx, B[DB_SEGS].ensure(nseg + 16)); HIPCHK(ctx, B[DB_SEGP].ensure(nseg * 4 + 16));
        HIPCHK(ctx, hipMemsetAsync(B[DB_SEGN].p, 0, (size_t)n_chunks * nstr * 4, A));
#define RFQ_SUM_ARGS a->d_rfq, CH, D, R, (const uint64_t*)qbase, (const uint64_t*)sbase, qdec, sdec, B[DB_SEGF].as<uint8_t>(), B[DB_SEGA].as<int>(), B[DB_SEGN].as<uint32_t>(), maxseg, dst, (uint64_t)a->n
        if (nn) hipLaunchKernelGGL(k_dec_pos_sum, dim3(mq, nn, n_chunks), dim3(64), 0, A, RFQ_SUM_ARGS, 0u, nstr);
        if (hasn) hipLaunchKernelGGL(k_dec_pos_sum, dim3(mn, 1, n_chunks), dim3(64), 0, A, RFQ_SUM_ARGS, HH.n_normal, nstr);
#undef RFQ_SUM_ARGS
        hipLaunchKernelGGL(k_dec_pos_link, dim3((n_chunks * nstr + 255) / 256), dim3(256), 0, A, (const uint8_t*)B[DB_SEGF].as<uint8_t>(),
                (const int*)B[DB_SEGA].as<int>(),
                           (const uint32_t*)B[DB_SEGN].as<uint32_t>(), B[DB_SEGS].as<uint8_t>(), B[DB_SEGP].as<int>(), maxseg, n_chunks * nstr);
        if (forked) { HIPCHK(ctx, hipEventRecord(ctx->ev_mid, A)); HIPCHK(ctx, hipStreamWaitEvent(S, ctx->ev_mid, 0)); HIPCHK(ctx, hipStreamWaitEvent(S, ctx->ev_f, 0)); }
        hipLaunchKernelGGL(k_dec_unpack, dim3(bpc, n_chunks), dim3(256), 0, A, a->d_rfq, CH, R, (const uint64_t*)sbase, sdec, (uint64_t)a->n);
        if (nn) hipLaunchKernelGGL(k_dec_pos_emit, dim3(mq, nn, n_chunks), dim3(64), 0, S, a->d_rfq, CH, D, R, (const uint64_t*)qbase, (const uint64_t*)sbase, qdec, sdec,
                                   (const uint8_t*)B[DB_SEGS].as<uint8_t>(), (const int*)B[DB_SEGP].as<int>(), maxseg, (uint64_t)a->n, 0u, nstr);
        if (hasn) hipLaunchKernelGGL(k_dec_pos_emit, dim3(mn, 1, n_chunks), dim3(64), 0, A, a->d_rfq, CH, D, R, (const uint64_t*)qbase, (const uint64_t*)sbase, qdec,
                sdec,
                                     (const uint8_t*)B[DB_SEGS].as<uint8_t>(), (const int*)B[DB_SEGP].as<int>(), maxseg, (uint64_t)a->n, HH.n_normal, nstr);
    } else hipLaunchKernelGGL(k_dec_unpack, dim3(bpc, n_chunks), dim3(256), 0, A, a->d_rfq, CH, R, (const uint64_t*)sbase, sdec, (uint64_t)a->n);
    if (forked) { HIPCHK(ctx, hipEventRecord(ctx->ev_join, A)); HIPCHK(ctx, hipStreamWaitEvent(S, ctx->ev_join, 0)); HIPCHK(ctx, hipStreamWaitEvent(S, ctx->ev_f, 0)); }
    if (rle_h) hipLaunchKernelGGL(k_dec_rle, dim3(1, n_chunks), dim3(256), 0, S, a->d_rfq, CH, D, R, (const uint64_t*)qbase, qdec);
    hipLaunchKernelGGL(k_dec_except, dim3(bpc, n_chunks), dim3(256), 0, S, a->d_rfq, CH, D, R, (const uint64_t*)qbase, qdec);
    KCHK(ctx, "k_dec_streams");
    ctx->timer.end(S);
    E->qbase = qbase; E->sbase = sbase; E->qdec = qdec; E->sdec = sdec; E->qbytes = qbytes; E->sbytes = sbytes;
    return RFQ_OK;
}
struct FusedPlan { bool on; uint32_t e3k; bool n1big, shared_pieces; };
static FusedPlan plan_fused(const rfq_ctx* ctx, const DecRange& g, bool force_expanded) {
    const DevHeader& HH = ctx->h_hdr;
    const bool rle_h = !(HH.flags & (H_DONT_QUAL | H_QUAL_BY_COL));
    uint32_t e3k = 6; bool n1big = false;
    while (e3k >= 1 && ((uint64_t)g.max_len << e3k) > E3_QCAP) e3k--;
    if (g.pieces) {
        while (e3k >= 1 && ((uint64_t)g.piece_avg << e3k) > 204u) e3k--;
        const uint64_t need1 = ((uint64_t)g.piece_n1 << e3k) * 5u / 4u + 32u;
        if (need1 > ET_N1CAP) { if (e3k == 6 && need1 <= E3_N1BIG) n1big = true; else e3k = 0; }
    }
    const bool e3_ok = e3k >= (g.pieces ? 6u : 1u) && !(g.pieces && ctx->e3_pieces_failed);
    const bool on = !force_expanded && !ctx->opt.materialise && !rle_h && g.max_len <= 2000u && g.max_nrec <= 4096u && e3_ok && g.max_bases < (1u << 30) - 65536u;
    return { on, e3k, n1big, E3_SHARED_OK && !g.pieces && !(HH.flags & H_DONT_QUAL) };
}
struct ListChain { uint32_t maxseg = 1, ncell = 1, nstr = 1, mq = 0, mn = 0, nn = 0, segb = POS2_SEG; bool hasn = false, built = false, join = false; hipStream_t aux = nullptr; };
struct AuxJoin { rfq_ctx* c; bool armed; ~AuxJoin() { if (armed) (void)hipStreamSynchronize(c->aux); } };

static void launch_pos_list(rfq_ctx* ctx, const rfq_decode_args* a, const DecRange& g, const ListChain& L, hipStream_t LS) {
    DBuf* B = ctx->b; const DevHeader* D = ctx->d_hdr.as<DevHeader>(); const DecStatus* dst = B[DB_STATUS].as<DecStatus>();
    const unsigned long long cap = B[DB_PLIST].cap / sizeof(plist_t);
#define RFQ_LIST_ARGS a->d_rfq, g.CH, D, (const uint8_t*)B[DB_SEGS].as<uint8_t>(), (const int*)B[DB_SEGP].as<int>(), (const uint32_t*)B[DB_SEGK].as<uint32_t>(), \
                      (const unsigned long long*)B[DB_LOFF].as<unsigned long long>(), B[DB_PLIST].as<plist_t>(), cap, B[DB_CELL].as<uint32_t>(), L.maxseg, L.ncell, (uint64_t)a->n
    if (L.nn) hipLaunchKernelGGL(k_dec_pos_list, dim3((L.mq + 3) / 4, L.nn, g.n_chunks), dim3(256), 0, LS, RFQ_LIST_ARGS, 0u, L.nstr, dst, L.segb);
    if (L.hasn) hipLaunchKernelGGL(k_dec_pos_list, dim3((L.mn + 3) / 4, 1, g.n_chunks), dim3(256), 0, LS, RFQ_LIST_ARGS, ctx->h_hdr.n_normal, L.nstr, dst, L.segb);
#undef RFQ_LIST_ARGS
}
static int dec_list_chain(rfq_ctx* ctx, const rfq_decode_args* a, const DecRange& g, AuxJoin& guard, ListChain* L) {
    hipStream_t S = ctx->stream; DBuf* B = ctx->b; const DevHeader& HH = ctx->h_hdr; const DevHeader* D = ctx->d_hdr.as<DevHeader>();
    DecStatus* dst = B[DB_STATUS].as<DecStatus>(); const DChunk* CH = g.CH; const uint32_t n_chunks = g.n_chunks;
    const bool bycol_h = (HH.flags & H_QUAL_BY_COL) && !(HH.flags & H_DONT_QUAL);
    L->nstr = HH.n_normal + 1; L->hasn = (HH.flags & H_N_POS) != 0; L->nn = bycol_h ? std::min<uint32_t>(HH.n_normal, NPOS_SLOT) : 0u;
    if (!L->nn && !L->hasn) return RFQ_OK;
    const bool forked = ctx->aux_ready(); hipStream_t A = forked ? ctx->aux : S;
    if (forked) { HIPCHK(ctx, hipEventRecord(ctx->ev_fork, S)); HIPCHK(ctx, hipStreamWaitEvent(A, ctx->ev_fork, 0)); guard.armed = true; }
    L->segb = ctx->opt.pos_seg ? (uint32_t)ctx->opt.pos_seg : (std::max(g.max_one, g.max_npos) >= 32768u ? POS2_SEG_BIG : POS2_SEG);
    L->mq = L->nn ? g.max_one / L->segb + 1 : 0u; L->mn = L->hasn ? g.max_npos / L->segb + 1 : 0u; L->maxseg = std::max(1u, std::max(L->mq, L->mn));
    L->ncell = g.max_bases / POS2_CELL + 2;
    const size_t nst = (size_t)n_chunks * L->nstr, nseg = nst * L->maxseg, ncl = nst * L->ncell;
    HIPCHK(ctx, B[DB_SEGF].ensure(nseg + 16)); HIPCHK(ctx, B[DB_SEGA].ensure(nseg * 32 + 16)); HIPCHK(ctx, B[DB_SEGN].ensure(nst * 4 + 16));
    HIPCHK(ctx, B[DB_SEGS].ensure(nseg + 16)); HIPCHK(ctx, B[DB_SEGP].ensure(nseg * 4 + 16)); HIPCHK(ctx, B[DB_SEGK].ensure(nseg * 4 + 16));
    HIPCHK(ctx, B[DB_CELL].ensure(ncl * 4 + 16));
    HIPCHK(ctx, B[DB_NENT].ensure(nst * 4 + 16)); HIPCHK(ctx, B[DB_LOFF].ensure(nst * 8 + 16));
    if (B[DB_PLIST].ensure((size_t)(g.bases / 8 + 1024) * sizeof(plist_t)) != hipSuccess) { (void)hipGetLastError();
            HIPCHK(ctx, B[DB_PLIST].ensure((size_t)(g.bases / 32 + 1024) * sizeof(plist_t))); }
    { ClearList z; memset(&z, 0, sizeof z); z.add(B[DB_SEGN].p, nst * 4, 0u); z.add(B[DB_NENT].p, nst * 4, 0u); z.add(B[DB_CELL].p, ncl * 4, 0xFFFFFFFFu); clear_list(A, z); }
#define RFQ_SUM2_ARGS a->d_rfq, CH, D, B[DB_SEGF].as<uint8_t>(), B[DB_SEGA].as<int>(), B[DB_SEGN].as<uint32_t>(), L->maxseg, dst, (uint64_t)a->n
    if (L->nn) hipLaunchKernelGGL(k_dec_pos_sum2, dim3((L->mq + 3) / 4, L->nn, n_chunks), dim3(256), 0, A, RFQ_SUM2_ARGS, 0u, L->nstr, L->segb);
    if (L->hasn) hipLaunchKernelGGL(k_dec_pos_sum2, dim3((L->mn + 3) / 4, 1, n_chunks), dim3(256), 0, A, RFQ_SUM2_ARGS, HH.n_normal, L->nstr, L->segb);
#undef RFQ_SUM2_ARGS
    hipLaunchKernelGGL(k_dec_pos_link2, dim3((uint32_t)((nst + 3) / 4)), dim3(256), 0, A, (const uint8_t*)B[DB_SEGF].as<uint8_t>(), (const int*)B[DB_SEGA].as<int>(),
                       (const uint32_t*)B[DB_SEGN].as<uint32_t>(), B[DB_SEGS].as<uint8_t>(), B[DB_SEGP].as<int>(), B[DB_SEGK].as<uint32_t>(), B[DB_NENT].as<uint32_t>(),
                       L->maxseg, (uint32_t)nst, CH, L->nstr, dst);
    hipLaunchKernelGGL(k_dec_pos_off, dim3(1), dim3(256), 0, A, (const uint32_t*)B[DB_NENT].as<uint32_t>(), B[DB_LOFF].as<unsigned long long>(), (uint32_t)nst, dst);
    launch_pos_list(ctx, a, g, *L, A);
    L->built = true; L->join = forked; L->aux = A;
    KCHK(ctx, "k_dec_pos_*");
    return RFQ_OK;
}
static int dec_table_fused(rfq_ctx* ctx, const rfq_decode_args* a, const DecRange& g, const FusedPlan& P, const DReadTab& R, DFused* F) {
    hipStream_t S = ctx->stream; DBuf* B = ctx->b;
    const size_t nr = (size_t)g.n_reads + 2, nc = (size_t)g.n_chunks + 2;
    HIPCHK(ctx, B[DB_PQL].ensure((nr + nc) * 4)); HIPCHK(ctx, B[DB_TPL].ensure(nr * 8));
    if (!P.shared_pieces) HIPCHK(ctx, B[DB_PVL].ensure((nr + nc) * 16));
    HIPCHK(ctx, B[DB_CTEXT].ensure(nc * 16)); HIPCHK(ctx, B[DB_TBASE].ensure(nc * 16)); HIPCHK(ctx, B[DB_SCAN].ensure((nc / SCAN_TILE + 2) * 16 + 1024));
    HIPCHK(ctx, B[DB_SDL].ensure((nr + nc) * 4));
    U4* const pvl = P.shared_pieces ? (U4*)nullptr : B[DB_PVL].as<U4>();
    F->len = R.len; F->ov = R.ov; F->pql = B[DB_PQL].as<uint32_t>(); F->pvl = pvl; F->sdl = B[DB_SDL].as<uint32_t>();
    F->tpl = B[DB_TPL].as<uint2>(); F->tbase = B[DB_TBASE].as<U4>(); F->mid = R.mid;
    hipLaunchKernelGGL(k_dec_readtab2, dim3(g.n_chunks), dim3(256), 0, S, a->d_rfq, g.CH, ctx->d_hdr.as<DevHeader>(), R.len, R.ov, B[DB_PQL].as<uint32_t>(), pvl,
                       B[DB_SDL].as<uint32_t>(), B[DB_STATUS].as<DecStatus>());
    KCHK(ctx, "k_dec_readtab2");
    ctx->timer.end(S);
    return RFQ_OK;
}
static int dec_textlen_fused(rfq_ctx* ctx, const rfq_decode_args* a, const DecRange& g, const DReadTab& R) {
    hipStream_t S = ctx->stream; DBuf* B = ctx->b; const DevHeader* D = ctx->d_hdr.as<DevHeader>();
    ctx->timer.begin("streams", S);
    hipLaunchKernelGGL(k_dec_coords, dim3(2, g.n_chunks), dim3(64), 0, S, a->d_rfq, g.CH, D, B[DB_XV].as<uint32_t>(), B[DB_YV].as<uint32_t>());
    KCHK(ctx, "k_dec_coords");
    hipLaunchKernelGGL(k_dec_textlen2, dim3(g.n_chunks), dim3(256), 0, S, a->d_rfq, g.CH, D, (const uint32_t*)R.len, R.mid, (const uint32_t*)B[DB_XV].as<uint32_t>(),
                       (const uint32_t*)B[DB_YV].as<uint32_t>(), a->split_pe ? 1 : 0, B[DB_TPL].as<uint2>(), B[DB_CTEXT].as<U4>(), B[DB_STATUS].as<DecStatus>());
    KCHK(ctx, "k_dec_textlen2");
    scan_exclusive<U4>(S, B[DB_CTEXT].as<U4>(), B[DB_TBASE].as<U4>(), g.n_chunks, B[DB_SCAN].as<U4>(), 1);
    return RFQ_OK;
}
static void launch_emit3(rfq_ctx* ctx, const rfq_decode_args* a, const DecRange& g, const FusedPlan& P, const ListChain& L, const DFused& F,
                         uint8_t* o1, uint64_t cap1, uint8_t* o2, uint64_t cap2, unsigned long long list_cap) {
    DBuf* B = ctx->b; const bool hasn = (ctx->h_hdr.flags & H_N_POS) != 0;
    const uint32_t K = 1u << P.e3k, bx = grid_x_for(g.n_chunks, (std::max(g.max_reads, 1u) + K - 1) / K, (P.n1big ? 4u : 6u) * ctx->n_cu);
    const dim3 grid(bx, g.n_chunks);
#define RFQ_EMIT3_ARGS a->d_rfq, g.CH, ctx->d_hdr.as<DevHeader>(), F, (uint64_t)a->n, a->split_pe ? 1 : 0, o1, cap1, o2, cap2, B[DB_STATUS].as<DecStatus>(), \
                       (const plist_t*)B[DB_PLIST].as<plist_t>(), (const unsigned long long*)B[DB_LOFF].as<unsigned long long>(), (const uint32_t*)B[DB_NENT].as<uint32_t>(), \
                       (const uint32_t*)B[DB_CELL].as<uint32_t>(), L.ncell, L.nstr, P.e3k, list_cap
    if (P.n1big) {
        if (hasn) hipLaunchKernelGGL((k_dec_emit3<false, E3_N1BIG>), grid, dim3(256), 0, ctx->stream, RFQ_EMIT3_ARGS);
        else hipLaunchKernelGGL((k_dec_emit3<true, E3_N1BIG>), grid, dim3(256), 0, ctx->stream, RFQ_EMIT3_ARGS);
    } else if (F.pvl == nullptr) {
        if (hasn) hipLaunchKernelGGL((k_dec_emit3<false, ET_N1CAP, true>), grid, dim3(256), 0, ctx->stream, RFQ_EMIT3_ARGS);
        else hipLaunchKernelGGL((k_dec_emit3<true, ET_N1CAP, true>), grid, dim3(256), 0, ctx->stream, RFQ_EMIT3_ARGS);
    }
    else if (hasn) hipLaunchKernelGGL(k_dec_emit3<false>, grid, dim3(256), 0, ctx->stream, RFQ_EMIT3_ARGS);
    else hipLaunchKernelGGL(k_dec_emit3<true>, grid, dim3(256), 0, ctx->stream, RFQ_EMIT3_ARGS);
#undef RFQ_EMIT3_ARGS
}
static int decode_range(rfq_ctx* ctx, const rfq_decode_args* a, const DecRange& g, uint8_t* out1, uint64_t ocap1, uint8_t* out2, uint64_t ocap2,
                        uint8_t** p1, uint8_t** p2, size_t* n1, size_t* n2, uint64_t* nbases, bool force_expanded = false) {
    hipStream_t S = ctx->stream; DBuf* B = ctx->b; const DevHeader* D = ctx->d_hdr.as<DevHeader>();
    DecStatus* dst = B[DB_STATUS].as<DecStatus>(); DecStatus hs;
    const uint32_t n_chunks = g.n_chunks, n_reads = g.n_reads, max_reads = std::max(g.max_reads, 1u);
    const int split = a->split_pe ? 1 : 0;
    HIPCHK(ctx, hipMemsetAsync(dst, 0, sizeof(DecStatus), S));
    const FusedPlan P = plan_fused(ctx, g, force_expanded);
    ListChain L; AuxJoin aux_guard = { ctx, false };
    if (P.on) { const int rc = dec_list_chain(ctx, a, g, aux_guard, &L); if (rc) return rc; }
    ctx->timer.begin("read_table", S);
    const size_t nr = (size_t)n_reads + 2;
    HIPCHK(ctx, B[DB_LEN].ensure(nr * 4)); HIPCHK(ctx, B[DB_OV].ensure(nr * 4));
    HIPCHK(ctx, B[DB_XV].ensure(nr * 4)); HIPCHK(ctx, B[DB_YV].ensure(nr * 4)); HIPCHK(ctx, B[DB_MID].ensure(nr * 40));
    DReadTab R; memset(&R, 0, sizeof R); DFused F; memset(&F, 0, sizeof F); DecExpanded E; memset(&E, 0, sizeof E);
    R.len = B[DB_LEN].as<uint32_t>(); R.ov = B[DB_OV].as<int32_t>(); R.mid = B[DB_MID].as<uint8_t>();
    if (P.on) {
        int rc = dec_table_fused(ctx, a, g, P, R, &F);
        if (!rc) rc = dec_textlen_fused(ctx, a, g, R);
        if (rc) return rc;
        *nbases = g.bases;
    } else {
        uint32_t total_bases = 0; U4 pv_tot; memset(&pv_tot, 0, sizeof pv_tot);
        int rc = dec_table_expanded(ctx, a, g, R, true, &total_bases, &pv_tot);
        if (!rc) rc = dec_streams_expanded(ctx, a, g, R, total_bases, pv_tot, true, &E);
        if (rc) return rc;
        *nbases = total_bases;
        ctx->timer.begin("textlen", S);
        hipLaunchKernelGGL(k_dec_textlen, dim3((max_reads + 255) / 256, n_chunks), dim3(256), 0, S, a->d_rfq, g.CH, D, R, (const uint32_t*)B[DB_XV].as<uint32_t>(),
                           (const uint32_t*)B[DB_YV].as<uint32_t>(), split, dst);
        scan_exclusive<U4>(S, R.tin, R.tp, n_reads, B[DB_SCAN].as<U4>(), 1);
    }
    if (L.join) { HIPCHK(ctx, hipEventRecord(ctx->ev_join, L.aux)); HIPCHK(ctx, hipStreamWaitEvent(S, ctx->ev_join, 0)); }
    aux_guard.armed = false;
    bool emitted = P.on && L.built && out1 && (!a->split_pe || out2) && !((uintptr_t)out1 & 15u) && !(out2 && ((uintptr_t)out2 & 15u)) && !ctx->opt.no_spec;
    if (emitted) {
        ctx->timer.end(S);
        ctx->timer.begin("emit", S);
        launch_emit3(ctx, a, g, P, L, F, out1, ocap1, out2, ocap2, B[DB_PLIST].cap / sizeof(plist_t));
        KCHK(ctx, "k_dec_emit");
        ctx->timer.end(S);
    }
    U4 tt; HIPCHK(ctx, ctx->fetch(&tt, P.on ? B[DB_TBASE].as<U4>() + n_chunks : R.tp + n_reads, 16, S));
    uint8_t *o1, *o2;
    for (;;) {
        HIPCHK(ctx, ctx->fetch(&hs, dst, sizeof hs, S));
        HIPCHK(ctx, ctx->fetch_sync(S));
        if (hs.err & DE_CORRUPT_OV) return rfq_fail(ctx, RFQ_E_FORMAT, "corrupt overlap buffer");
        if (P.on && (hs.err & (DE_LIST_ALIAS | DE_E3_RETRY))) {
            if ((hs.err & DE_E3_RETRY) && g.pieces) ctx->e3_pieces_failed = true;
            return decode_range(ctx, a, g, out1, ocap1, out2, ocap2, p1, p2, n1, n2, nbases, true);
        }
        if (hs.err & DE_CORRUPT) return rfq_fail(ctx, RFQ_E_FORMAT, "corrupt quality buffer");
        if (L.built && hs.list_need > B[DB_PLIST].cap / sizeof(plist_t)) {
            if (emitted) { emitted = false; ctx->timer.begin("streams", S); }
            HIPCHK(ctx, B[DB_PLIST].ensure((size_t)(hs.list_need + 1024) * sizeof(plist_t)));
            launch_pos_list(ctx, a, g, L, S);
            KCHK(ctx, "k_dec_pos_list");
        }
        hs.text1 = hs.text2 = 0; for (int i = 0; i < 64; i++) { hs.text1 += hs.text_slots[0][i]; hs.text2 += hs.text_slots[1][i]; }
        if (hs.text1 >= 0xFFFFFFF0ull || hs.text2 >= 0xFFFFFFF0ull) return RFQ_RANGE_TOO_BIG;
        if ((out1 && ((uintptr_t)out1 & 15u)) || (out2 && ((uintptr_t)out2 & 15u))) return rfq_fail(ctx, RFQ_E_ARG, "output device pointers must be 16-byte aligned");
        uint64_t cap1, cap2;
        if (out1) { o1 = out1; cap1 = ocap1; } else { HIPCHK(ctx, ctx->out_fq1.ensure((size_t)tt.a + 64)); o1 = ctx->out_fq1.as<uint8_t>(); cap1 = ctx->out_fq1.cap; }
        if (out2) { o2 = out2; cap2 = ocap2; } else { HIPCHK(ctx, ctx->out_fq2.ensure((size_t)tt.b + 64)); o2 = ctx->out_fq2.as<uint8_t>(); cap2 = ctx->out_fq2.cap; }
        if (emitted) break;
        ctx->timer.end(S);
        ctx->timer.begin(P.on ? "emit" : "emit_expanded", S);
        if (P.on) launch_emit3(ctx, a, g, P, L, F, o1, cap1, o2, cap2, 0ull);
        else {
            const uint32_t bx = grid_x_for(n_chunks, (max_reads + ET_READS - 1) / ET_READS, 4u * ctx->n_cu);
            hipLaunchKernelGGL(k_dec_emit, dim3(bx, n_chunks), dim3(256), 0, S, a->d_rfq, g.CH, D, R, (const uint64_t*)E.qbase, (const uint64_t*)E.sbase,
                               (const uint8_t*)E.qdec, (const uint8_t*)E.sdec, (uint64_t)E.qbytes, (uint64_t)E.sbytes, (uint64_t)a->n, split, o1, cap1, o2, cap2, dst);
        }
        KCHK(ctx, "k_dec_emit");
        ctx->timer.end(S);
        emitted = true;
    }
    ctx->timer.collect();
    if (hs.err & (1u << 31)) return rfq_fail(ctx, RFQ_E_NOSPACE, "output buffer too small: need %u / %u bytes", tt.a, tt.b);
    *n1 = tt.a; *n2 = split ? tt.b : 0; *p1 = o1; *p2 = o2;
    return RFQ_OK;
}

static DecRange range_of(const DecStatus& hs, const DChunk* CH, uint32_t n_chunks, uint64_t reads, uint64_t bases) {
    DecRange g; g.CH = CH; g.n_chunks = n_chunks; g.n_reads = (uint32_t)reads; g.max_reads = hs.max_reads; g.max_stream = hs.max_stream;
            g.max_npos = hs.max_npos; g.max_len = hs.max_len; g.max_bases = hs.max_bases; g.max_nrec = hs.max_nrec; g.max_one = hs.max_one;
            g.pieces = hs.per_read_pieces; g.piece_avg = hs.piece_avg; g.piece_n1 = hs.piece_n1; g.bases = bases;
    return g;
}
struct ChunkSpan { uint32_t c0, c1; bool r1_only; };
static std::vector<ChunkSpan> plan_ranges(const std::vector<ChunkSpan>& pieces, const std::vector<DChunk>& hc, uint64_t slice_bases) {
    std::vector<ChunkSpan> fw, todo;
    for (auto& pc : pieces) {
        uint32_t c0 = pc.c0; uint64_t acc = 0, rd = 0;
        for (uint32_t c = pc.c0; c < pc.c1; c++) {
            if (c > c0 && (acc + hc[c].bases > slice_bases || rd + hc[c].reads > 0x7FFFFFF0ull)) { fw.push_back({ c0, c, pc.r1_only }); c0 = c; acc = 0; rd = 0; }
            acc += hc[c].bases; rd += hc[c].reads;
        }
        fw.push_back({ c0, pc.c1, pc.r1_only });
    }
    for (size_t i = fw.size(); i-- > 0;) todo.push_back(fw[i]);
    return todo;
}
static int span_range(rfq_ctx* ctx, const DecStatus& hs, DChunk* CHm, const std::vector<DChunk>& hc, const ChunkSpan& r, DecRange* g, uint64_t* reads) {
    uint64_t rd = 0, rbases = 0; for (uint32_t c = r.c0; c < r.c1; c++) { rd += hc[c].reads; rbases += hc[c].bases; }
    hipLaunchKernelGGL(k_dec_rebase, dim3((r.c1 - r.c0 + 255) / 256), dim3(256), 0, ctx->stream, CHm + r.c0, r.c1 - r.c0, hc[r.c0].rbase_abs);
    KCHK(ctx, "k_dec_rebase");
    *g = range_of(hs, CHm + r.c0, r.c1 - r.c0, rd, rbases); *reads = rd;
    return RFQ_OK;
}

static int dec_open(rfq_ctx* ctx, const rfq_decode_args* a, uint64_t* start) {
    HIPCHK(ctx, hipSetDevice(ctx->device));
    ctx->timer.reset();
    ctx->pend.clear(); ctx->pin_used = 0;
    *start = 0;
    if (a->has_header) {
        uint8_t hb[RFQ_HEADER_MAX]; const size_t take = std::min<size_t>(a->n, sizeof hb);
        if (take) HIPCHK(ctx, hipMemcpy(hb, a->d_rfq, take, hipMemcpyDeviceToHost));
        int rc = rfq_upload_header(ctx, hb, take);
        if (rc) return rc;
        *start = ctx->h_hdr.len;
    } else if (!ctx->have_hdr) return rfq_fail(ctx, RFQ_E_STATE, "decode without a header: pass has_header=1 or call rfq_set_header first");
    return RFQ_OK;
}
static int dec_walk(rfq_ctx* ctx, const rfq_decode_args* a, uint64_t start, DecStatus& hs) {
    hipStream_t S = ctx->stream; DBuf* B = ctx->b; const DevHeader& HH = ctx->h_hdr;
    if (HH.read_len_bytes != 1 && HH.read_len_bytes != 2 && HH.read_len_bytes != 4) return rfq_fail(ctx, RFQ_E_DATA,
            "header incorrect: read length bytes should be 1/2/4");
    const DevHeader* D = ctx->d_hdr.as<DevHeader>();

    ctx->timer.begin("walk", S);
    HIPCHK(ctx, B[DB_STATUS].ensure(sizeof(DecStatus)));
    DecStatus* dst = B[DB_STATUS].as<DecStatus>();
    uint32_t cap = (uint32_t)std::max<size_t>(B[DB_CHUNKS].cap / sizeof(DChunk), 4096);
    bool use_table = a->h_chunk_off && a->n_chunk_off && a->h_chunk_off[0] == start && a->h_chunk_off[a->n_chunk_off] <= a->n;
    bool guess = !use_table && !ctx->opt.walk_exact;
    for (;;) {
        if (use_table && a->n_chunk_off + 1u > cap) cap = a->n_chunk_off + 1u;
        HIPCHK(ctx, B[DB_CHUNKS].ensure((size_t)cap * sizeof(DChunk)));
        ClearList wz; memset(&wz, 0, sizeof wz); wz.add(dst, sizeof(DecStatus), 0u);
        const bool indexed = use_table || guess;
        if (use_table) {
            const size_t tb = ((size_t)a->n_chunk_off + 1) * 8;
            clear_list(S, wz);
            HIPCHK(ctx, B[DB_OFFT].ensure(tb));
            HIPCHK(ctx, hipMemcpyAsync(B[DB_OFFT].p, a->h_chunk_off, tb, hipMemcpyHostToDevice, S));
            hipLaunchKernelGGL(k_dec_table, dim3(1), dim3(256), 0, S, a->d_rfq, (uint64_t)a->n, (const uint64_t*)B[DB_OFFT].as<uint64_t>(), a->n_chunk_off,
                    B[DB_CHUNKS].as<DChunk>(), dst);
        } else if (guess) {
            HIPCHK(ctx, B[DB_OFFT].ensure(((size_t)cap + 2) * 8));
            HIPCHK(ctx, B[DB_GWCAND].ensure(GW_SEGS * 8 + 64)); HIPCHK(ctx, B[DB_GWLIST].ensure((size_t)GW_SEGS * GW_LCAP * 8));
                    HIPCHK(ctx, B[DB_GWCNT].ensure(GW_SEGS * 4 + 64)); HIPCHK(ctx, B[DB_GWLAND].ensure(GW_SEGS * 8 + 64));
            unsigned long long* cand = B[DB_GWCAND].as<unsigned long long>(); uint32_t* gbad = B[DB_GWCNT].as<uint32_t>() + GW_SEGS;
            wz.add(cand, GW_SEGS * 8, 0xFFFFFFFFu); wz.add(gbad, 4, 0u); clear_list(S, wz);
            const uint32_t mseg = (uint32_t)std::min<uint64_t>(GW_SEGS, std::max<uint64_t>(1, (a->n - start) >> ctx->opt.gw_shift));
            if (mseg > 1) hipLaunchKernelGGL(k_dec_gw_find, dim3(16, mseg - 1), dim3(256), 0, S, a->d_rfq, (uint64_t)a->n, start, D, cand, mseg);
            hipLaunchKernelGGL(k_dec_gw_walk, dim3(mseg), dim3(64), 0, S, a->d_rfq, (uint64_t)a->n, start, D, (const unsigned long long*)cand,
                    B[DB_GWLIST].as<unsigned long long>(), B[DB_GWCNT].as<uint32_t>(), B[DB_GWLAND].as<unsigned long long>(), gbad, mseg, a->final ? 1 : 0);
            hipLaunchKernelGGL(k_dec_gw_stitch, dim3(1), dim3(1024), 0, S, a->d_rfq, (uint64_t)a->n, start, D, (const unsigned long long*)cand,
                    (const unsigned long long*)B[DB_GWLIST].as<unsigned long long>(),
                               (const uint32_t*)B[DB_GWCNT].as<uint32_t>(), (const unsigned long long*)B[DB_GWLAND].as<unsigned long long>(), (const uint32_t*)gbad, B[DB_OFFT].as<uint64_t>(), cap, dst, mseg);
            hipLaunchKernelGGL(k_dec_table, dim3(1), dim3(256), 0, S, a->d_rfq, (uint64_t)a->n, (const uint64_t*)B[DB_OFFT].as<uint64_t>(), 0xFFFFFFFFu,
                    B[DB_CHUNKS].as<DChunk>(), dst);
        }
        else { clear_list(S, wz); hipLaunchKernelGGL(k_dec_walk, dim3(1), dim3(64), 0, S, a->d_rfq, (uint64_t)a->n, start, D, B[DB_CHUNKS].as<DChunk>(), cap, dst, a->final ? 1 : 0); }
        KCHK(ctx, "k_dec_walk");
        const uint32_t PARSE_AHEAD = use_table ? std::max(a->n_chunk_off, 1u) : 4096u;
        if (indexed) {
            hipLaunchKernelGGL(k_dec_parse, dim3(std::min(cap, PARSE_AHEAD)), dim3(64), 0, S, a->d_rfq, (uint64_t)a->n, D, B[DB_CHUNKS].as<DChunk>(), dst, 0u);
            hipLaunchKernelGGL(k_dec_summary, dim3(1), dim3(256), 0, S, (const DChunk*)B[DB_CHUNKS].as<DChunk>(), dst, 0u, std::min(cap, PARSE_AHEAD));
            KCHK(ctx, "k_dec_parse");
        }
        HIPCHK(ctx, ctx->fetch(&hs, dst, sizeof hs, S));
        HIPCHK(ctx, ctx->fetch_sync(S));
        if (use_table) {
            if (hs.pad || (hs.consumed != a->n && a->n - hs.consumed >= 18 && (a->final || hs.n_chunks == 0))) { use_table = false; guess = !ctx->opt.walk_exact;
                    continue; }
            break;
        }
        if (hs.overflow) { cap = hs.n_chunks + 1024; continue; }
        if (!indexed) { hs.max_nrec = 0xFFFFFFFFu; hs.max_one = hs.max_stream; hs.per_read_pieces = 1; hs.piece_avg = 0xFFFFu; hs.piece_n1 = 0xFFFFu; break; }
        if (hs.pad) { guess = false; continue; }
        if (hs.n_chunks > PARSE_AHEAD) {
            hipLaunchKernelGGL(k_dec_parse, dim3(hs.n_chunks - PARSE_AHEAD), dim3(64), 0, S, a->d_rfq, (uint64_t)a->n, D, B[DB_CHUNKS].as<DChunk>(), dst, PARSE_AHEAD);
            hipLaunchKernelGGL(k_dec_summary, dim3(1), dim3(256), 0, S, (const DChunk*)B[DB_CHUNKS].as<DChunk>(), dst, PARSE_AHEAD, hs.n_chunks - PARSE_AHEAD);
            KCHK(ctx, "k_dec_parse");
            DecStatus h2; HIPCHK(ctx, ctx->fetch(&h2, dst, sizeof h2, S));
            HIPCHK(ctx, ctx->fetch_sync(S));
            if (h2.pad) { guess = false; continue; }
            hs.max_stream = h2.max_stream; hs.max_npos = h2.max_npos; hs.max_len = h2.max_len; hs.max_bases = h2.max_bases; hs.max_nrec = h2.max_nrec;
                    hs.max_one = h2.max_one; hs.per_read_pieces = h2.per_read_pieces; hs.piece_avg = h2.piece_avg; hs.piece_n1 = h2.piece_n1;
                    memcpy(hs.base_slots, h2.base_slots, sizeof hs.base_slots);
        }
        if (hs.consumed != a->n && a->n - hs.consumed >= 18 && (a->final || hs.n_chunks == 0)) { guess = false; continue; }
        break;
    }
    if (ctx->opt.trace) fprintf(stderr, "[rfq] chunk starts: %s, %u chunks\n", use_table ? "caller's index" : (guess ? "guess-and-verify" : "exact walk"), hs.n_chunks);
    ctx->timer.end(S);
    if (hs.err & DE_CORRUPT) return rfq_fail(ctx, RFQ_E_FORMAT, "truncated or corrupt rfq chunk at byte %llu", (unsigned long long)hs.consumed);
    return RFQ_OK;
}

extern "C" int rfq_decode_batch(rfq_ctx* ctx, const rfq_decode_args* a, rfq_decode_result* res) {
    if (!ctx || !a || !res) return RFQ_E_ARG;
    memset(res, 0, sizeof *res);
    ctx->err.clear();
    if (a->n && !a->d_rfq) return rfq_fail(ctx, RFQ_E_ARG, "null rfq pointer");
    if (a->n == 0 && a->has_header) {
        if (a->split_pe) return rfq_fail(ctx, RFQ_E_DATA, "The input RFQ file was encoded by single-end FASTQ, you should not specify <out2>");
        return RFQ_OK;
    }
    uint64_t start = 0;
    { const int rc = dec_open(ctx, a, &start); if (rc) return rc; }
    const DevHeader& HH = ctx->h_hdr;
    if (a->split_pe && !(HH.flags & H_PAIRED)) return rfq_fail(ctx, RFQ_E_DATA, "The input RFQ file was encoded by single-end FASTQ, you should not specify <out2>");
    DecStatus hs;
    { const int rc = dec_walk(ctx, a, start, hs); if (rc) return rc; }
    DBuf* B = ctx->b; hipStream_t S = ctx->stream;
    uint64_t tb = 0; for (int i = 0; i < 16; i++) tb += hs.base_slots[i];
    const uint32_t n_chunks = hs.n_chunks; const uint64_t n_reads64 = hs.total_reads;
    res->consumed = (size_t)hs.consumed; res->n_chunks = n_chunks; res->n_reads = n_reads64;
    if (n_chunks == 0) return RFQ_OK;
    const uint32_t last_flags = hs.last_flags; const int split = a->split_pe ? 1 : 0;
    DChunk* CHm = B[DB_CHUNKS].as<DChunk>();
    const uint64_t slice_env = ctx->opt.slice_bases;
    const uint64_t slice_bases = slice_env ? slice_env : 1500000000ull, one_pass = slice_env ? slice_env : 0xFFFFFFF0ull;
    size_t n1 = 0, n2 = 0; uint64_t nb = 0; uint8_t *o1 = nullptr, *o2 = nullptr;
    int rc = RFQ_RANGE_TOO_BIG;
    std::vector<ChunkSpan> pieces; std::vector<DChunk> hc; bool strip1 = (last_flags & C_NO_LB) != 0, strip2 = (last_flags & C_NO_LB_R2) != 0;
    const bool compat = a->bug_compat != 0 && split;
    if (compat) {
        hc.resize(n_chunks);
        HIPCHK(ctx, hipMemcpy(hc.data(), CHm, (size_t)n_chunks * sizeof(DChunk), hipMemcpyDeviceToHost));
        uint32_t run = 0, end = n_chunks; strip1 = strip2 = false;
        for (uint32_t i = 0; i < n_chunks;) {
            const bool f1 = (hc[i].flags & C_NO_LB) != 0, f2 = split && (hc[i].flags & C_NO_LB_R2) != 0;
            if (!f1 && !f2) { i++; continue; }
            if (i + 1 == n_chunks) {
                if (!a->final) { end = i; res->consumed = (size_t)hc[i].off; }
                else { strip1 = f1; strip2 = f2; }
                break;
            }
            if (split && f1) { if (i > run) pieces.push_back({ run, i, false }); pieces.push_back({ i, i + 1, true }); }
            else pieces.push_back({ run, i + 1, false });
            run = i + 2; i += 2;
        }
        if (run < end) pieces.push_back({ run, end, false });
        res->n_chunks = 0; for (auto& q : pieces) res->n_chunks += q.c1 - q.c0;
    }
    if (!compat && tb < one_pass && n_reads64 < 0x7FFFFFF0ull) {
        const DecRange g = range_of(hs, CHm, n_chunks, n_reads64, tb);
        rc = decode_range(ctx, a, g, a->d_out1, a->cap1, a->d_out2, a->cap2, &o1, &o2, &n1, &n2, &nb);
        if (rc != RFQ_OK && rc != RFQ_RANGE_TOO_BIG) return rc;
    }
    if (rc == RFQ_RANGE_TOO_BIG) {
        if (!compat) { hc.resize(n_chunks); HIPCHK(ctx, hipMemcpy(hc.data(), CHm, (size_t)n_chunks * sizeof(DChunk), hipMemcpyDeviceToHost));
                pieces.push_back({ 0, n_chunks, false }); }
        std::vector<ChunkSpan> todo = plan_ranges(pieces, hc, slice_bases);
        size_t w1 = 0, w2 = 0; n1 = n2 = 0; nb = 0;
        StageSums sums; ctx->timer.collect(); sums.add(ctx->timer);
        while (!todo.empty()) {
            const ChunkSpan r = todo.back(); todo.pop_back();
            DecRange g; uint64_t reads = 0;
            rc = span_range(ctx, hs, CHm, hc, r, &g, &reads);
            if (rc) return rc;
            uint8_t *q1 = nullptr, *q2 = nullptr; size_t m1 = 0, m2 = 0; uint64_t mb = 0;
            ctx->timer.reset();
            rc = reads > 0x7FFFFFF0ull ? RFQ_RANGE_TOO_BIG : decode_range(ctx, a, g, nullptr, 0, nullptr, 0, &q1, &q2, &m1, &m2, &mb);
            if (rc == RFQ_RANGE_TOO_BIG) {
                if (r.c1 - r.c0 < 2) return rfq_fail(ctx, RFQ_E_ARG, "a single chunk decodes to 4 GiB of text or more");
                const uint32_t mid = r.c0 + (r.c1 - r.c0) / 2; todo.push_back({ mid, r.c1, r.r1_only }); todo.push_back({ r.c0, mid, r.r1_only }); continue;
            }
            if (rc != RFQ_OK) return rc;
            sums.add(ctx->timer);
            for (int k = 0; k < (split ? 2 : 1); k++) {
                uint8_t* src = k ? q2 : q1; const size_t m = k ? m2 : m1; size_t& w = k ? w2 : w1; uint8_t* dcall = k ? a->d_out2 : a->d_out1;
                        const size_t dcap = k ? a->cap2 : a->cap1;
                if (!m || (k && r.r1_only)) continue;
                uint8_t* to;
                if (dcall) { if (w + m > dcap) return rfq_fail(ctx, RFQ_E_NOSPACE, "output buffer too small"); to = dcall + w; }
                else { DBuf& ab = k ? ctx->out_acc2 : ctx->out_acc1; HIPCHK(ctx, ab.ensure_keep(w + m + 64, w, S)); to = ab.as<uint8_t>() + w; }
                HIPCHK(ctx, hipMemcpyAsync(to, src, m, hipMemcpyDeviceToDevice, S));
                w += m;
            }
            HIPCHK(ctx, hipStreamSynchronize(S));
            nb += mb;
        }
        n1 = w1; n2 = w2;
        o1 = a->d_out1 ? a->d_out1 : ctx->out_acc1.as<uint8_t>(); o2 = a->d_out2 ? a->d_out2 : ctx->out_acc2.as<uint8_t>();
        sums.publish(ctx->timer);
    }
    res->n_bases = nb;
    if (a->final) {
        if (strip1 && n1) n1--;
        if (split && strip2 && n2) n2--;
    }
    res->d_fq1 = o1; res->n1 = n1; res->d_fq2 = split ? o2 : nullptr; res->n2 = split ? n2 : 0;
    return RFQ_OK;
}

static int rows_range(rfq_ctx* ctx, const rfq_decode_args* a, const DecRange& g, const RowsOut& o) {
    hipStream_t S = ctx->stream; DBuf* B = ctx->b; const DevHeader* D = ctx->d_hdr.as<DevHeader>(); DecStatus* dst = B[DB_STATUS].as<DecStatus>();
    HIPCHK(ctx, hipMemsetAsync(dst, 0, sizeof(DecStatus), S));
    ctx->timer.begin("read_table", S);
    const size_t nr = (size_t)g.n_reads + 2;
    HIPCHK(ctx, B[DB_LEN].ensure(nr * 4)); HIPCHK(ctx, B[DB_OV].ensure(nr * 4));
    DReadTab R; memset(&R, 0, sizeof R); R.len = B[DB_LEN].as<uint32_t>(); R.ov = B[DB_OV].as<int32_t>();
    uint32_t total_bases = 0; U4 pv_tot; memset(&pv_tot, 0, sizeof pv_tot);
    int rc = dec_table_expanded(ctx, a, g, R, false, &total_bases, &pv_tot);
    if (rc) return rc;
    DecExpanded E; rc = dec_streams_expanded(ctx, a, g, R, total_bases, pv_tot, false, &E);
    if (rc) return rc;
    DecStatus h; HIPCHK(ctx, ctx->fetch(&h, dst, sizeof h, S)); HIPCHK(ctx, ctx->fetch_sync(S));
    if (h.err & DE_CORRUPT) return rfq_fail(ctx, RFQ_E_FORMAT, "corrupt quality buffer");
    ctx->timer.begin("rows", S);
    const uint32_t bx = grid_x_for(g.n_chunks, (std::max(g.max_reads, 1u) + 31u) / 32u, 8u * ctx->n_cu);
    hipLaunchKernelGGL(k_dec_rows, dim3(bx, g.n_chunks), dim3(256), 0, S, g.CH, (const DevHeader*)D, R, (const uint64_t*)E.qbase, (const uint64_t*)E.sbase,
                       (const uint8_t*)E.qdec, (const uint8_t*)E.sdec, o);
    KCHK(ctx, "k_dec_rows");
    ctx->timer.end(S);
    HIPCHK(ctx, hipStreamSynchronize(S));
    return RFQ_OK;
}

extern "C" int rfq_decode_rows(rfq_ctx* ctx, const rfq_decode_rows_args* ra, rfq_decode_rows_result* res) {
    if (!ctx || !ra || !res) return RFQ_E_ARG;
    memset(res, 0, sizeof *res);
    ctx->err.clear();
    if (ra->n && !ra->d_rfq) return rfq_fail(ctx, RFQ_E_ARG, "null rfq pointer");
    if (ra->base_mode != RFQ_ROWS_ASCII && ra->base_mode != RFQ_ROWS_CODE) return rfq_fail(ctx, RFQ_E_ARG, "base_mode must be RFQ_ROWS_ASCII or RFQ_ROWS_CODE");
    const bool query = !ra->d_bases && !ra->d_quals && !ra->d_lens;
    if (!query && ra->row_len == 0) return rfq_fail(ctx, RFQ_E_ARG, "row_len must be at least 1");
    if ((uintptr_t)ra->d_lens & 3u) return rfq_fail(ctx, RFQ_E_ARG, "d_lens must be 4-byte aligned");
    rfq_decode_args a; memset(&a, 0, sizeof a);
    a.d_rfq = ra->d_rfq; a.n = ra->n; a.has_header = ra->has_header; a.final = ra->final; a.h_chunk_off = ra->h_chunk_off; a.n_chunk_off = ra->n_chunk_off;
    if (a.n == 0 && a.has_header) return RFQ_OK;
    uint64_t start = 0;
    { const int rc = dec_open(ctx, &a, &start); if (rc) return rc; }
    DecStatus hs;
    { const int rc = dec_walk(ctx, &a, start, hs); if (rc) return rc; }
    hipStream_t S = ctx->stream;
    uint64_t tb = 0; for (int i = 0; i < 16; i++) tb += hs.base_slots[i];
    const uint32_t n_chunks = hs.n_chunks; const uint64_t n_rows = n_chunks ? hs.total_reads : 0;
    res->consumed = (size_t)hs.consumed; res->n_chunks = n_chunks; res->n_rows = n_rows; res->n_bases = n_chunks ? tb : 0; res->max_len = n_chunks ? hs.max_len : 0;
    if (query || n_chunks == 0) { HIPCHK(ctx, hipStreamSynchronize(S)); ctx->timer.collect(); return RFQ_OK; }
    const uint64_t L = ra->row_len, need = n_rows * L;
    if (L < res->max_len) return rfq_fail(ctx, RFQ_E_NOSPACE, "row_len %u is shorter than the longest read: need row_len >= %u", ra->row_len, res->max_len);
    if (ra->d_bases && ra->bases_cap < need) return rfq_fail(ctx, RFQ_E_NOSPACE, "base rows too small: need %llu bytes (%llu rows of %u)", (unsigned long long)need,
            (unsigned long long)n_rows, ra->row_len);
    if (ra->d_quals && ra->quals_cap < need) return rfq_fail(ctx, RFQ_E_NOSPACE, "quality rows too small: need %llu bytes (%llu rows of %u)", (unsigned long long)need,
            (unsigned long long)n_rows, ra->row_len);
    if (ra->d_lens && ra->lens_cap < n_rows) return rfq_fail(ctx, RFQ_E_NOSPACE, "length array too small: need %llu entries", (unsigned long long)n_rows);
    RowsOut o; memset(&o, 0, sizeof o);
    o.bases = ra->d_bases; o.quals = ra->d_quals; o.lens = ra->d_lens; o.row_len = L; o.n_rows = n_rows;
    o.codes = ra->base_mode == RFQ_ROWS_CODE ? 1u : 0u;
    o.qoff4 = ra->qual_offset * 0x01010101u; o.pad_b4 = ra->pad_base * 0x01010101u; o.pad_q4 = ra->pad_qual * 0x01010101u;
    o.vec = (L % 16u == 0 && !((uintptr_t)ra->d_bases & 15u) && !((uintptr_t)ra->d_quals & 15u)) ? 1u : 0u;
    DChunk* CHm = ctx->b[DB_CHUNKS].as<DChunk>();
    const uint64_t slice_env = ctx->opt.slice_bases;
    const uint64_t slice_bases = slice_env ? slice_env : 1500000000ull, one_pass = slice_env ? slice_env : 0xFFFFFFF0ull;
    if (tb < one_pass && n_rows < 0x7FFFFFF0ull) {
        const int rc = rows_range(ctx, &a, range_of(hs, CHm, n_chunks, n_rows, tb), o);
        if (rc) return rc;
        ctx->timer.collect();
        return RFQ_OK;
    }
    std::vector<DChunk> hc(n_chunks);
    HIPCHK(ctx, hipMemcpy(hc.data(), CHm, (size_t)n_chunks * sizeof(DChunk), hipMemcpyDeviceToHost));
    std::vector<ChunkSpan> todo = plan_ranges(std::vector<ChunkSpan>{ { 0, n_chunks, false } }, hc, slice_bases);
    HIPCHK(ctx, hipStreamSynchronize(S));
    StageSums sums; ctx->timer.collect(); sums.add(ctx->timer);
    while (!todo.empty()) {
        const ChunkSpan r = todo.back(); todo.pop_back();
        DecRange g; uint64_t reads = 0;
        int rc = span_range(ctx, hs, CHm, hc, r, &g, &reads);
        if (rc) return rc;
        if (g.bases >= 0xFFFFFFF0ull || reads >= 0x7FFFFFF0ull) return rfq_fail(ctx, RFQ_E_ARG, "a single chunk holds 4 Gi bases or 2 Gi reads or more");
        ctx->timer.reset();
        rc = rows_range(ctx, &a, g, o);
        if (rc) return rc;
        ctx->timer.collect(); sums.add(ctx->timer);
    }
    sums.publish(ctx->timer);
    return RFQ_OK;
}
```

Before: 1.099 million MB/s.

## Build read-name mid fields in LDS inside emit kernel instead of global buffer

The textlen kernel no longer writes the 32-byte per-read formatted lane/tile/x/y row to a global mid buffer; it only computes digit lengths. The fused emit kernel now formats these rows directly into double-buffered shared memory from the x/y coordinate arrays, prefetching names one tile ahead and L2-prefetching x/y two tiles ahead. This removes a global write and read of 32 bytes per read, in exchange for extra integer formatting work inside the emit kernel and an extra LDS buffer when prefetch is off. A selftest entry point for the mid formatting helpers is also added.

```diff
diff --git a/include/rfq_hip.h b/include/rfq_hip.h
--- a/include/rfq_hip.h
+++ b/include/rfq_hip.h
@@ -163,6 +163,8 @@
 
 RFQ_API int rfq_selftest_wave(rfq_ctx* ctx, const uint64_t* h_in, uint32_t n_waves, uint64_t* h_out);
 
+RFQ_API int rfq_selftest_mid(rfq_ctx* ctx, const uint32_t* h_val, const uint32_t* h_off, uint32_t n, uint32_t* h_out);
+
 RFQ_API const char* rfq_version(void);
 
 #ifdef __cplusplus
diff --git a/repaq_amd/_capi.py b/repaq_amd/_capi.py
--- a/repaq_amd/_capi.py
+++ b/repaq_amd/_capi.py
@@ -119,6 +119,8 @@
     L.rfq_get_option.argtypes = [C.c_void_p, C.c_char_p, C.c_char_p, C.c_size_t]
     L.rfq_option_name.argtypes = [C.c_int]; L.rfq_option_name.restype = C.c_char_p
     L.rfq_selftest_wave.argtypes = [C.c_void_p, C.POINTER(C.c_uint64), C.c_uint32, C.POINTER(C.c_uint64)]
+    if hasattr(L, "rfq_selftest_mid"):
+        L.rfq_selftest_mid.argtypes = [C.c_void_p, C.POINTER(C.c_uint32), C.POINTER(C.c_uint32), C.c_uint32, C.POINTER(C.c_uint32)]
     _libs[path] = L
     return L
 
@@ -126,4 +128,4 @@
 EXPORTS = ["rfq_version", "rfq_create", "rfq_destroy", "rfq_last_error", "rfq_set_stream", "rfq_set_header", "rfq_get_header", "rfq_clear_header",
            "rfq_encode_batch", "rfq_scan_batch", "rfq_decode_batch", "rfq_decode_rows", "rfq_rows_to_text", "rfq_encode_rows", "rfq_last_timings", "rfq_dev_malloc", "rfq_dev_free", "rfq_copy_h2d", "rfq_copy_d2h",
            "rfq_copy_h2d_async", "rfq_copy_done", "rfq_copy_sync",
-           "rfq_copy_d2d", "rfq_copy_peer", "rfq_host_alloc", "rfq_host_free", "rfq_compare_bytes", "rfq_selftest_wave", "rfq_set_option", "rfq_get_option", "rfq_option_name", "rfq_host_register", "rfq_host_unregister"]
+           "rfq_copy_d2d", "rfq_copy_peer", "rfq_host_alloc", "rfq_host_free", "rfq_compare_bytes", "rfq_selftest_wave", "rfq_selftest_mid", "rfq_set_option", "rfq_get_option", "rfq_option_name", "rfq_host_register", "rfq_host_unregister"]
diff --git a/repaq_amd/codec.py b/repaq_amd/codec.py
--- a/repaq_amd/codec.py
+++ b/repaq_amd/codec.py
@@ -64,6 +64,13 @@
         a = (C.c_uint64 * n)(*lanes); o = (C.c_uint64 * (12 * n))()
         self._check(self._L.rfq_selftest_wave(self._h, a, n // 64, o))
         return [list(o[12 * i: 12 * i + 12]) for i in range(n)]
+
+    def selftest_mid(self, vals, offs):
+        n = len(vals); assert n and n == len(offs)
+        a = (C.c_uint32 * n)(*vals); k = (C.c_uint32 * n)(*offs); o = (C.c_uint32 * (12 * n))()
+        self._check(self._L.rfq_selftest_mid(self._h, a, k, n, o))
+        raw = bytes(o)
+        return [(o[12 * i], o[12 * i + 1], raw[48 * i + 8: 48 * i + 48]) for i in range(n)]
 
     def setHeader(self, header_bytes: bytes):
         self._check(self._L.rfq_set_header(self._h, header_bytes, len(header_bytes)))
diff --git a/repaq_amd/csrc/dec/emit_tiles.h b/repaq_amd/csrc/dec/emit_tiles.h
--- a/repaq_amd/csrc/dec/emit_tiles.h
+++ b/repaq_amd/csrc/dec/emit_tiles.h
@@ -47,7 +47,7 @@
     constexpr uint32_t NB = (SHARED && E3_PREFETCH) ? 2u : 1u;
     __shared__ uint4 t_pk4[NB][E3_QCAP / 64 + 6];
     __shared__ uint32_t t_nb[E3_QCAP / 32 + 8];
-    __shared__ uint4 t_mid4_[NB][64 * E3_MIDROW / 16 + 5], t_n14_[(SHARED ? 256u : N1CAP) / 16 + 5], t_n24_[(SHARED ? 256u : ET_N2CAP) / 16 + 5], t_st4[(SHARED ? 256u : ET_STCAP) / 16 + 4];
+    __shared__ uint4 t_mid4_[2][64 * E3_MIDROW / 16 + 5], t_n14_[(SHARED ? 256u : N1CAP) / 16 + 5], t_n24_[(SHARED ? 256u : ET_N2CAP) / 16 + 5], t_st4[(SHARED ? 256u : ET_STCAP) / 16 + 4];
     uint4* const t_n14 = t_n14_ + 1; uint4* const t_n24 = t_n24_ + 1;
     __shared__ unsigned long long s_loff[NPOS_SLOT + 2]; __shared__ uint32_t s_nent[NPOS_SLOT + 2], s_val[NPOS_SLOT + 2];
     __shared__ uint32_t s_g[2][NPOS_SLOT + 2], s_kb[2][NPOS_SLOT + 2];
@@ -118,13 +118,27 @@
     auto tile_fits = [&](const TileP& tp) -> bool {
         return tp.q1 - tp.q0 <= E3_QCAP && (same1 || tp.e7 - tp.a7 + 32u <= N1CAP) && (same2 || tp.e8 - tp.a8 + 32u <= ET_N2CAP) && (same3 || tp.e9 - tp.a9 + 32u <= ET_STCAP);
     };
-    auto stage = [&](const TileD& t, uint32_t g0_, uint32_t g1_, uint32_t bsel) {
+    auto stage = [&](const TileD& t, uint32_t bsel) {
         if (raw) span_dma<(int)((E3_QCAP / 16 + 4 + 255) / 256)>(make_span(t_q4 + 1, img, t.rqa, t.rqe, img_bytes, true));
         if (w == 0) span_dma_wave<(int)((E3_QCAP / 64 + 4 + 63) / 64), PF>(make_span(t_pk4[bsel], img, t.pka, t.pke, img_bytes, true), l);
-        else if (w == 1) span_dma_wave<(int)((64 * E3_MIDROW / 16 + 4 + 63) / 64), PF>(make_span(t_mid4_[bsel] + 1, F.mid, (uint64_t)g0_ * E3_MIDROW, (uint64_t)g1_ * E3_MIDROW, ~0ull >> 1, true), l);
         else if (w == 2) { if (!same1) span_dma_wave<(int)((N1CAP / 16 + 4 + 63) / 64)>(make_span(t_n14, img, t.n1a, t.n1e, img_bytes, true), l); }
         else { if (!same2) span_dma_wave<(int)((ET_N2CAP / 16 + 4 + 63) / 64)>(make_span(t_n24, img, t.n2a, t.n2e, img_bytes, true), l);
                if (!same3) span_dma_wave<(int)((ET_STCAP / 16 + 4 + 63) / 64)>(make_span(t_st4, img, t.sta, t.ste, img_bytes, true), l); }
+    };
+    auto load_names = [&](uint32_t cur_, uint32_t cnt_) -> DName {
+        DName nm; nm.n1 = nm.n2 = nm.st = nm.lane = nm.tile = nm.x = nm.y = 0;
+        if (w == 1 && (uint32_t)l < cnt_) nm = dec_name_parts(cp, d, D, F.xv, F.yv, cur_ + (uint32_t)l);
+        return nm;
+    };
+    auto put_mids = [&](const DName& nm, uint32_t cnt_, uint32_t bsel) {
+        if (w == 1 && (uint32_t)l < cnt_) {
+            uint8_t* const buf = (uint8_t*)(t_mid4_[bsel] + 1) + E3_MIDROW * (uint32_t)l; uint32_t k = 0;
+            { uint4* z = (uint4*)buf; z[0] = z[1] = make_uint4(0, 0, 0, 0); }
+            if (hf & H_LANE) k += mid_put(buf, k, E3_MIDROW, nm.lane);
+            if (hf & H_TILE) k += mid_put(buf, k, E3_MIDROW, nm.tile);
+            if (hf & H_X) k += mid_put(buf, k, E3_MIDROW, nm.x);
+            if (hf & H_Y) k += mid_put(buf, k, E3_MIDROW, nm.y);
+        }
     };
     struct ReadM { uint32_t len, md, prevlen, sdl, pql, tx; int ov; U4 p4; uint8_t n1, n2, sl; };
     auto load_read = [&](uint32_t cur_, uint32_t cnt_) -> ReadM {
@@ -165,19 +179,20 @@
         }
         return L;
     };
+    { const uint32_t cnt0 = re - cur < K ? re - cur : K; put_mids(load_names(cur, cnt0), cnt0, 0u); }
     __syncthreads();
     ReadM mN; ListS lN;
     if constexpr (PF) {
-        if (tile_fits(tp_cur)) { const uint32_t cnt0 = re - cur < K ? re - cur : K; stage(tile_spans(tp_cur), f + cur, f + cur + cnt0, 0u); mN = load_read(cur, cnt0); lN = load_lists(0u); }
+        if (tile_fits(tp_cur)) { const uint32_t cnt0 = re - cur < K ? re - cur : K; stage(tile_spans(tp_cur), 0u); mN = load_read(cur, cnt0); lN = load_lists(0u); }
         else { mN = load_read(cur, 0u); lN = load_lists(0u); }
     }
     while (cur < re) {
-        const uint32_t cnt = re - cur < K ? re - cur : K, g0 = f + cur, g1 = g0 + cnt;
+        const uint32_t cnt = re - cur < K ? re - cur : K;
         const TileP tp = tp_cur; const uint32_t q0 = tp.q0, q1 = tp.q1, s0 = tp.s0, s1 = tp.s1;
         if (!tile_fits(tp)) { if (tid == 0) atomicOr(&st->err, (uint32_t)DE_E3_RETRY); break; }
         const TileD td = tile_spans(tp); const uint32_t bs = PF ? pb : 0u;
         const uint64_t n1a = td.n1a, n2a = td.n2a, sta = td.sta, pka = td.pka, pke = td.pke, rqa = td.rqa;
-        if constexpr (!PF) { stage(td, g0, g1, 0u); mN = load_read(cur, cnt); lN = load_lists(pb); }
+        if constexpr (!PF) { stage(td, 0u); mN = load_read(cur, cnt); lN = load_lists(pb); }
         const ReadM m = mN; ListS ls = lN;
         if (bycol) { uint4* qt = t_q4 + 1; const uint32_t ng = (q1 - q0 + 15u) >> 4;
                 for (uint32_t i = tid; i < ng; i += blockDim.x) qt[i] = make_uint4(major4, major4, major4, major4); }
@@ -188,6 +203,8 @@
         if (on) { sp = m.sdl - s0; qp_ = m.pql - q0; toff = (to2 ? tb.b : tb.a) + m.tx; if constexpr (!SHARED) { o7 = m.p4.a - tp.a7; o8 = m.p4.b - tp.a8; o9 = m.p4.c - tp.a9; } }
         const uint32_t nxt = cur + cnt; TileP tp_n = tp;
         if (nxt < re) tp_n = tile_params(nxt, nxt + K < re ? nxt + K : re);
+        const uint32_t cntn = nxt < re ? (re - nxt < K ? re - nxt : K) : 0u;
+        const DName nmN = load_names(nxt, cntn);
 #ifndef RFQ_SIMT_EMULATION
         if constexpr (PF) __builtin_amdgcn_s_waitcnt(0x0F70);
 #endif
@@ -197,7 +214,7 @@
 #endif
         uint8_t* const q_t = (uint8_t*)(t_q4 + 1) + (raw ? (uint32_t)(rqa & 15ull) : 0u);
         const uint8_t* const pk = (const uint8_t*)t_pk4[bs] + (uint32_t)(pka & 15ull);
-        const uint4* const t_mid4 = t_mid4_[bs] + 1;
+        const uint4* const t_mid4 = t_mid4_[pb] + 1;
         const uint32_t have = (uint32_t)(pke - pka), sbit0 = 2u * (s0 & 3u);
         {
 #pragma unroll
@@ -222,19 +239,24 @@
         }
         if (nxt < re && tid < T) { s_g[pb ^ 1u][tid] = cell_lookup(tid, tp_n.q0, tp_n.s0, false); s_kb[pb ^ 1u][tid] = cell_lookup(tid, tp_n.q0, tp_n.s0, true); }
         __syncthreads();
+        put_mids(nmN, cntn, pb ^ 1u);
         if constexpr (PF) {
             if (nxt < re) {
-                const uint32_t cntn = re - nxt < K ? re - nxt : K;
-                if (tile_fits(tp_n)) { stage(tile_spans(tp_n), f + nxt, f + nxt + cntn, pb ^ 1u); mN = load_read(nxt, cntn); lN = load_lists(pb ^ 1u); }
+                if (tile_fits(tp_n)) { stage(tile_spans(tp_n), pb ^ 1u); mN = load_read(nxt, cntn); lN = load_lists(pb ^ 1u); }
             }
         }
 #if E3_L2PF && !defined(RFQ_SIMT_EMULATION)
         if (SHARED && nxt < re) {
-            const uint32_t cntn = re - nxt < K ? re - nxt : K; const TileD tn = tile_spans(tp_n);
+            const TileD tn = tile_spans(tp_n);
             const uint8_t* pb_ = nullptr; uint32_t nbytes = 0;
             const uint32_t grp = tid >> 5, li = tid & 31u; uint32_t line = li;
             if (grp == 0) { pb_ = img + tn.pka; nbytes = (uint32_t)(tn.pke - tn.pka); }
-            else if (grp == 1) { pb_ = F.mid + (size_t)(f + nxt) * E3_MIDROW; nbytes = cntn * E3_MIDROW; }
+            else if (grp == 1 && nxt + K < re) {
+                const uint32_t n2 = nxt + K, c2 = re - n2 < K ? re - n2 : K;
+                const uint32_t a = li >> 4, x0 = il ? n2 >> 1 : n2, xn = il ? (c2 + 1u) >> 1 : c2; line = li & 15u;
+                if (a == 0 && (hf & H_X)) { pb_ = (const uint8_t*)(F.xv + f + x0); nbytes = xn * 4u; }
+                else if (a == 1 && (hf & H_Y)) { pb_ = (const uint8_t*)(F.yv + f + x0); nbytes = xn * 4u; }
+            }
             else if (grp == 2) {
                 const uint32_t a = li >> 2; line = li & 3u;
                 if (a == 0) { pb_ = (const uint8_t*)(F.tpl + f + nxt); nbytes = cntn * 8u; }
@@ -263,7 +285,7 @@
             else {
                 const uint32_t L = e0 + 1u; const bool nfast = L >= 16u, jfast = sl == 1u && len >= 16u;
                 const uint8_t* const src1 = (const uint8_t*)t_n14 + (uint32_t)(n1a & 15ull) + (same1 ? 0u : o7);
-                const uint8_t* const src2 = (const uint8_t*)t_mid4 + (uint32_t)(((uint64_t)g0 * E3_MIDROW) & 15ull) + E3_MIDROW * j;
+                const uint8_t* const src2 = (const uint8_t*)t_mid4 + E3_MIDROW * j;
                 const uint8_t* const src3 = (const uint8_t*)t_n24 + (uint32_t)(n2a & 15ull) + (same2 ? 0u : o8);
                 const uint8_t* const src4 = (const uint8_t*)t_st4 + (uint32_t)(sta & 15ull) + (same3 ? 0u : o9);
                 const int pat2 = (same2 && rc && dch != 0 && dpos < n2) ? (int)dpos : -1;
diff --git a/repaq_amd/csrc/dec/read_table.h b/repaq_amd/csrc/dec/read_table.h
--- a/repaq_amd/csrc/dec/read_table.h
+++ b/repaq_amd/csrc/dec/read_table.h
@@ -34,7 +34,7 @@
     const uint32_t* sdl;
     const uint2* tpl;
     const U4* tbase;
-    const uint8_t* mid;
+    const uint32_t* xv; const uint32_t* yv;
 };
 __global__ void __launch_bounds__(256) k_dec_readtab2(const uint8_t* __restrict__ img, const DChunk* __restrict__ CH, const DevHeader* __restrict__ D,
                                                       uint32_t* __restrict__ len_o, int32_t* __restrict__ ov_o, uint32_t* __restrict__ pql, U4* __restrict__ pvl, uint32_t* __restrict__ sdl, DecStatus* st) {
diff --git a/repaq_amd/csrc/dec/text_len.h b/repaq_amd/csrc/dec/text_len.h
--- a/repaq_amd/csrc/dec/text_len.h
+++ b/repaq_amd/csrc/dec/text_len.h
@@ -13,6 +13,9 @@
     LdsU8 w; w.a = (asc << 8) | 0x3Aull; *(LdsU8*)(buf + k) = w;
     if (n == 8u) buf[k + 8u] = (uint8_t)(asc >> 56);
     return 1u + n;
+}
+__device__ __forceinline__ uint32_t mid_len(uint32_t v) {
+    return 2u + (v >= 10u) + (v >= 100u) + (v >= 1000u) + (v >= 10000u) + (v >= 100000u) + (v >= 1000000u) + (v >= 10000000u) + (v >= 100000000u) + (v >= 1000000000u);
 }
 struct DName { uint32_t n1, n2, st, lane, tile, x, y; };
 __device__ __forceinline__ DName dec_name_parts(const uint8_t* cp, const DChunk& d, const DevHeader* D, const uint32_t* xv, const uint32_t* yv, uint32_t r) {
@@ -65,9 +68,8 @@
     }
 }
 __global__ void __launch_bounds__(256) k_dec_textlen2(const uint8_t* __restrict__ img, const DChunk* __restrict__ CH, const DevHeader* __restrict__ D, const uint32_t* __restrict__ len_i,
-                                                      uint8_t* __restrict__ mid, const uint32_t* __restrict__ xv, const uint32_t* __restrict__ yv, int split,
+                                                      const uint32_t* __restrict__ xv, const uint32_t* __restrict__ yv, int split,
                                                       uint2* __restrict__ tpl, U4* __restrict__ ctext, DecStatus* st) {
-    __shared__ unsigned long long s_mid[256 * 4];
     const uint32_t c = blockIdx.x; const DChunk d = CH[c]; const uint8_t* cp = img + d.off; const uint32_t hf = D->flags;
     unsigned long long carry = 0, sum1 = 0, sum2 = 0;
     for (uint32_t r0 = 0; r0 < d.reads; r0 += blockDim.x) {
@@ -75,14 +77,10 @@
         if (r < d.reads) {
             const size_t g = (size_t)d.rbase + r;
             const DName m = dec_name_parts(cp, d, D, xv, yv, r);
-            uint8_t* buf = (uint8_t*)(s_mid + 4u * threadIdx.x);
-            { unsigned long long* z = (unsigned long long*)buf; z[0] = z[1] = z[2] = z[3] = 0ull; }
-            if (hf & H_LANE) k += mid_put(buf, k, E3_MIDROW, m.lane);
-            if (hf & H_TILE) k += mid_put(buf, k, E3_MIDROW, m.tile);
-            if (hf & H_X) k += mid_put(buf, k, E3_MIDROW, m.x);
-            if (hf & H_Y) k += mid_put(buf, k, E3_MIDROW, m.y);
-            { const unsigned long long* z = (const unsigned long long*)buf; unsigned long long* mp = (unsigned long long*)(mid + g * E3_MIDROW);
-              const unsigned long long a0 = z[0], a1 = z[1], a2 = z[2], a3 = z[3]; mp[0] = a0; mp[1] = a1; mp[2] = a2; mp[3] = a3; }
+            if (hf & H_LANE) k += mid_len(m.lane);
+            if (hf & H_TILE) k += mid_len(m.tile);
+            if (hf & H_X) k += mid_len(m.x);
+            if (hf & H_Y) k += mid_len(m.y);
             const uint32_t len = len_i[g]; const uint32_t text = m.n1 + m.n2 + k + 1 + len + 1 + m.st + 1 + len + 1;
             second = split && (r & 1u);
             mine = second ? ((unsigned long long)text << 32) : (unsigned long long)text;
diff --git a/repaq_amd/csrc/rfq_decode.hip b/repaq_amd/csrc/rfq_decode.hip
--- a/repaq_amd/csrc/rfq_decode.hip
+++ b/repaq_amd/csrc/rfq_decode.hip
@@ -157,7 +157,7 @@
     HIPCHK(ctx, B[DB_SDL].ensure((nr + nc) * 4));
     U4* const pvl = P.shared_pieces ? (U4*)nullptr : B[DB_PVL].as<U4>();
     F->len = R.len; F->ov = R.ov; F->pql = B[DB_PQL].as<uint32_t>(); F->pvl = pvl; F->sdl = B[DB_SDL].as<uint32_t>();
-    F->tpl = B[DB_TPL].as<uint2>(); F->tbase = B[DB_TBASE].as<U4>(); F->mid = R.mid;
+    F->tpl = B[DB_TPL].as<uint2>(); F->tbase = B[DB_TBASE].as<U4>(); F->xv = B[DB_XV].as<uint32_t>(); F->yv = B[DB_YV].as<uint32_t>();
     hipLaunchKernelGGL(k_dec_readtab2, dim3(g.n_chunks), dim3(256), 0, S, a->d_rfq, g.CH, ctx->d_hdr.as<DevHeader>(), R.len, R.ov, B[DB_PQL].as<uint32_t>(), pvl,
                        B[DB_SDL].as<uint32_t>(), B[DB_STATUS].as<DecStatus>());
     KCHK(ctx, "k_dec_readtab2");
@@ -169,7 +169,7 @@
     ctx->timer.begin("streams", S);
     hipLaunchKernelGGL(k_dec_coords, dim3(2, g.n_chunks), dim3(64), 0, S, a->d_rfq, g.CH, D, B[DB_XV].as<uint32_t>(), B[DB_YV].as<uint32_t>());
     KCHK(ctx, "k_dec_coords");
-    hipLaunchKernelGGL(k_dec_textlen2, dim3(g.n_chunks), dim3(256), 0, S, a->d_rfq, g.CH, D, (const uint32_t*)R.len, R.mid, (const uint32_t*)B[DB_XV].as<uint32_t>(),
+    hipLaunchKernelGGL(k_dec_textlen2, dim3(g.n_chunks), dim3(256), 0, S, a->d_rfq, g.CH, D, (const uint32_t*)R.len, (const uint32_t*)B[DB_XV].as<uint32_t>(),
                        (const uint32_t*)B[DB_YV].as<uint32_t>(), a->split_pe ? 1 : 0, B[DB_TPL].as<uint2>(), B[DB_CTEXT].as<U4>(), B[DB_STATUS].as<DecStatus>());
     KCHK(ctx, "k_dec_textlen2");
     scan_exclusive<U4>(S, B[DB_CTEXT].as<U4>(), B[DB_TBASE].as<U4>(), g.n_chunks, B[DB_SCAN].as<U4>(), 1);
@@ -207,7 +207,8 @@
     ctx->timer.begin("read_table", S);
     const size_t nr = (size_t)n_reads + 2;
     HIPCHK(ctx, B[DB_LEN].ensure(nr * 4)); HIPCHK(ctx, B[DB_OV].ensure(nr * 4));
-    HIPCHK(ctx, B[DB_XV].ensure(nr * 4)); HIPCHK(ctx, B[DB_YV].ensure(nr * 4)); HIPCHK(ctx, B[DB_MID].ensure(nr * 40));
+    HIPCHK(ctx, B[DB_XV].ensure(nr * 4)); HIPCHK(ctx, B[DB_YV].ensure(nr * 4));
+    if (!P.on) HIPCHK(ctx, B[DB_MID].ensure(nr * 40));
     DReadTab R; memset(&R, 0, sizeof R); DFused F; memset(&F, 0, sizeof F); DecExpanded E; memset(&E, 0, sizeof E);
     R.len = B[DB_LEN].as<uint32_t>(); R.ov = B[DB_OV].as<int32_t>(); R.mid = B[DB_MID].as<uint8_t>();
     if (P.on) {
@@ -581,3 +582,28 @@
     sums.publish(ctx->timer);
     return RFQ_OK;
 }
+
+__global__ void __launch_bounds__(64) k_selftest_mid(const uint32_t* __restrict__ val, const uint32_t* __restrict__ off, uint32_t n, uint32_t* __restrict__ out) {
+    __shared__ unsigned long long s_row[64 * 5];
+    const uint32_t i = blockIdx.x * 64u + threadIdx.x;
+    if (i >= n) return;
+    unsigned long long* const z = s_row + 5u * threadIdx.x; z[0] = z[1] = z[2] = z[3] = z[4] = 0xEEEEEEEEEEEEEEEEull;
+    const uint32_t v = val[i], k = off[i] <= 29u ? off[i] : 29u;
+    uint32_t* const o = out + 12u * (size_t)i;
+    o[0] = mid_len(v); o[1] = mid_put((uint8_t*)z, k, E3_MIDROW, v);
+    for (uint32_t j = 0; j < 5u; j++) { o[2u + 2u * j] = (uint32_t)z[j]; o[3u + 2u * j] = (uint32_t)(z[j] >> 32); }
+}
+extern "C" int rfq_selftest_mid(rfq_ctx* c, const uint32_t* h_val, const uint32_t* h_off, uint32_t n, uint32_t* h_out) {
+    if (!c || !h_val || !h_off || !h_out || !n) return RFQ_E_ARG;
+    HIPCHK(c, hipSetDevice(c->device));
+    uint32_t *dv = nullptr, *dk = nullptr, *dout = nullptr;
+    hipError_t e = hipMalloc((void**)&dv, (size_t)n * 4); if (e == hipSuccess) e = hipMalloc((void**)&dk, (size_t)n * 4); if (e == hipSuccess) e = hipMalloc((void**)&dout, (size_t)n * 48);
+    if (e == hipSuccess) e = hipMemcpy(dv, h_val, (size_t)n * 4, hipMemcpyHostToDevice);
+    if (e == hipSuccess) e = hipMemcpy(dk, h_off, (size_t)n * 4, hipMemcpyHostToDevice);
+    if (e == hipSuccess) { hipLaunchKernelGGL(k_selftest_mid, dim3((n + 63u) / 64u), dim3(64), 0, c->stream, (const uint32_t*)dv, (const uint32_t*)dk, n, dout); e = hipGetLastError(); }
+    if (e == hipSuccess) e = hipStreamSynchronize(c->stream);
+    if (e == hipSuccess) e = hipMemcpy(h_out, dout, (size_t)n * 48, hipMemcpyDeviceToHost);
+    (void)hipFree(dv); (void)hipFree(dk); (void)hipFree(dout);
+    if (e != hipSuccess) return rfq_fail(c, RFQ_E_HIP, "rfq_selftest_mid: %s", hipGetErrorString(e));
+    return RFQ_OK;
+}
```

Result: slower. 1.082 million MB/s (-1.5%).
